# Cheng-Lin-Li/show-attend-and-tell

Measured on AMD Instinct MI355X. Metric: training images/sec, higher is better.
Workload: dtype bf16; 1 GPU; model=vgg16_frozen+attention_lstm512, global_batch=32, seq_len=20, vocab=5000, parallelism=dp1

## Files before the change

### sat_amd/models/encoders.py

```python

import torch
import torch.nn as tnn

from .nn import BatchNorm, Conv2d, MaxPool2d


class VGG16(tnn.Module):
    _PLAN = [
        ('conv1_1', 64), ('conv1_2', 64), 'pool',
        ('conv2_1', 128), ('conv2_2', 128), 'pool',
        ('conv3_1', 256), ('conv3_2', 256), ('conv3_3', 256), 'pool',
        ('conv4_1', 512), ('conv4_2', 512), ('conv4_3', 512), 'pool',
        ('conv5_1', 512), ('conv5_2', 512), ('conv5_3', 512),
    ]

    num_ctx = 196
    dim_ctx = 512

    def __init__(self, nn_policy):
        super().__init__()
        layers = []
        in_ch = 3
        for item in self._PLAN:
            if item == 'pool':
                layers.append(MaxPool2d(2, 2))
            else:
                name, out_ch = item
                conv = Conv2d(nn_policy, in_ch, out_ch, 3, 1, 'relu')
                self.add_module(name, conv)
                layers.append(conv)
                in_ch = out_ch
        self._layers = layers
        self.conv1_1._emit_padded = True
        self.conv1_2._accept_padded = True

    def forward(self, images):
        x = images
        for layer in self._layers:
            x = layer(x)
        return x.permute(0, 2, 3, 1).reshape(
            x.shape[0], -1, x.shape[1]).contiguous()


class _Bottleneck(tnn.Module):
    def __init__(self, nn_policy, in_ch, mid_ch, stride, project):
        super().__init__()
        out_ch = mid_ch * 4
        self.project = project
        if project:
            self.shortcut = Conv2d(nn_policy, in_ch, out_ch, 1, stride,
                                   None, use_bias=False)
            self.shortcut_bn = BatchNorm(nn_policy, out_ch)
        self.conv_a = Conv2d(nn_policy, in_ch, mid_ch, 1, stride, None,
                             use_bias=False)
        self.bn_a = BatchNorm(nn_policy, mid_ch)
        self.conv_b = Conv2d(nn_policy, mid_ch, mid_ch, 3, 1, None,
                             use_bias=False)
        self.bn_b = BatchNorm(nn_policy, mid_ch)
        self.conv_c = Conv2d(nn_policy, mid_ch, out_ch, 1, 1, None,
                             use_bias=False)
        self.bn_c = BatchNorm(nn_policy, out_ch)

    def forward(self, x):
        if self.project:
            sc = self.shortcut_bn(self.shortcut(x))
        else:
            sc = x
        y = self.bn_a(self.conv_a(x), relu=True)
        y = self.bn_b(self.conv_b(y), relu=True)
        y = self.bn_c(self.conv_c(y))
        return torch.relu(y + sc)


class ResNet50(tnn.Module):
    _STAGES = [(64, 3, 1), (128, 4, 2), (256, 6, 2), (512, 3, 2)]

    num_ctx = 49
    dim_ctx = 2048

    def __init__(self, nn_policy):
        super().__init__()
        self.conv1 = Conv2d(nn_policy, 3, 64, 7, 2, None, use_bias=False)
        self.bn1 = BatchNorm(nn_policy, 64)
        self.pool1 = MaxPool2d(3, 2)
        blocks = []
        in_ch = 64
        for s, (mid, n, stride) in enumerate(self._STAGES, start=2):
            for b in range(n):
                blk = _Bottleneck(nn_policy, in_ch, mid,
                                  stride if b == 0 else 1, b == 0)
                self.add_module('res%d%s' % (s, chr(ord('a') + b)), blk)
                blocks.append(blk)
                in_ch = mid * 4
        self._blocks = blocks

    def forward(self, images):
        x = self.bn1(self.conv1(images), relu=True)
        x = self.pool1(x)
        for blk in self._blocks:
            x = blk(x)
        return x.permute(0, 2, 3, 1).reshape(
            x.shape[0], -1, x.shape[1]).contiguous()


def build_encoder(name, nn_policy):
    if name == 'vgg16':
        return VGG16(nn_policy)
    if name == 'resnet50':
        return ResNet50(nn_policy)
    raise ValueError('unknown cnn %r' % (name,))
```

### sat_amd/models/nn.py

```python

import math

import torch
import torch.nn as tnn

from .. import ops


class NN(object):

    def __init__(self, config):
        self.config = config
        self.is_train = getattr(config, 'phase', 'train') == 'train'
        self.train_cnn = self.is_train and getattr(config, 'train_cnn', False)
        self.fc_scale = config.fc_kernel_initializer_scale
        self.fc_reg = config.fc_kernel_regularizer_scale \
            if self.is_train else 0.0
        self.conv_reg = config.conv_kernel_regularizer_scale \
            if self.train_cnn else 0.0
        self.fc_drop_rate = config.fc_drop_rate
        self.lstm_drop_rate = config.lstm_drop_rate
        self.fc_act_reg = getattr(
            config, 'fc_activity_regularizer_scale', 0.0) \
            if self.is_train else 0.0
        self.conv_act_reg = getattr(
            config, 'conv_activity_regularizer_scale', 0.0) \
            if self.train_cnn else 0.0
        self._regularized = []
        self._act_losses = []

    def init_fc_(self, t):
        tnn.init.uniform_(t, -self.fc_scale, self.fc_scale)

    def init_conv_(self, t):
        tnn.init.xavier_uniform_(t)

    def register_fc_kernel(self, p):
        if self.fc_reg > 0:
            self._regularized.append((p, self.fc_reg))

    def register_conv_kernel(self, p):
        if self.conv_reg > 0:
            self._regularized.append((p, self.conv_reg))

    def add_activity_loss(self, y, scale):
        if scale > 0 and torch.is_grad_enabled():
            self._act_losses.append(scale * y.float().abs().sum())

    def reg_loss(self):
        total = torch.zeros(())
        if self._regularized:
            if self._regularized[0][0].is_cuda:
                params = tuple(p for p, _ in self._regularized)
                scales = tuple(s for _, s in self._regularized)
                total = _RegL2.apply(scales, *params)
            else:
                total = sum(s * 0.5 * (p.float() ** 2).sum()
                            for p, s in self._regularized)
        if self._act_losses:
            act = sum(self._act_losses)
            self._act_losses = []
            total = total.to(act.device) + act
        return total

    def dropout(self, x):
        return ops.dropout(x, self.fc_drop_rate, self.is_train)


class _RegL2(torch.autograd.Function):

    _scale_cache = {}

    @staticmethod
    def forward(ctx, scales, *params):
        ctx.save_for_backward(*params)
        ctx.scales = scales
        norms = torch._foreach_norm(params, 2)
        sv = torch.stack([n.float() for n in norms])
        key = (scales, sv.device)
        sc = _RegL2._scale_cache.get(key)
        if sc is None:
            sc = torch.tensor(scales, dtype=torch.float32,
                              device=sv.device)
            _RegL2._scale_cache[key] = sc
        return (sv * sv * sc * 0.5).sum()

    @staticmethod
    def backward(ctx, d):
        params = ctx.saved_tensors
        gs = torch._foreach_mul(params, list(ctx.scales))
        gs = torch._foreach_mul(gs, d)
        return (None, *gs)


class Dense(tnn.Module):

    def __init__(self, nn_policy, in_dim, units, activation='tanh',
                 use_bias=True):
        super().__init__()
        self.activation = activation
        self._nn = nn_policy
        self.weight = tnn.Parameter(torch.empty(units, in_dim))
        nn_policy.init_fc_(self.weight)
        nn_policy.register_fc_kernel(self.weight)
        if use_bias:
            self.bias = tnn.Parameter(torch.zeros(units))
        else:
            self.register_parameter('bias', None)
        self._wc = None
        self._bc = None

    def precast(self, dtype):
        self._wc = self.weight.to(dtype)
        self._bc = self.bias.to(dtype) if self.bias is not None else None

    def clear_cast(self):
        self._wc = None
        self._bc = None

    def forward(self, x):
        if self._wc is not None and self._wc.dtype == x.dtype:
            y = ops.dense(x, self._wc, self._bc, self.activation)
        else:
            w = self.weight.to(x.dtype)
            b = self.bias.to(x.dtype) if self.bias is not None else None
            y = ops.dense(x, w, b, self.activation)
        if self.activation is not None and self._nn.fc_act_reg > 0:
            self._nn.add_activity_loss(y, self._nn.fc_act_reg)
        return y


class Conv2d(tnn.Module):

    def __init__(self, nn_policy, in_ch, out_ch, kernel_size=3, stride=1,
                 activation='relu', use_bias=True):
        super().__init__()
        self.stride = stride
        self.kernel_size = kernel_size
        self.activation = activation
        self._nn = nn_policy
        self._glds_conv = getattr(nn_policy.config, 'use_glds_conv',
                                  True)
        self.weight = tnn.Parameter(
            torch.empty(out_ch, in_ch, kernel_size, kernel_size))
        nn_policy.init_conv_(self.weight)
        nn_policy.register_conv_kernel(self.weight)
        if use_bias:
            self.bias = tnn.Parameter(torch.zeros(out_ch))
        else:
            self.register_parameter('bias', None)

    def forward(self, x):
        w = self.weight.to(x.dtype)
        b = self.bias.to(x.dtype) if self.bias is not None else None
        k, st = self.kernel_size, self.stride
        pad_hw = getattr(x, '_sat_pad', None)
        if pad_hw is not None and not (
                getattr(self, '_accept_padded', False)
                and k == 3 and st == 1
                and not torch.is_grad_enabled()):
            x = x[:, :, 1:-1, 1:-1] \
                .contiguous(memory_format=torch.channels_last)
            pad_hw = None
        if (torch.is_grad_enabled()
                and (x.requires_grad or w.requires_grad)
                and self._glds_conv and k == 3 and st == 1
                and self.activation in ('relu', None)):
            from ..ops.convgrad import Conv3x3Train, conv3x3_train_ok
            if conv3x3_train_ok(x, w):
                y = Conv3x3Train.apply(x, w, b,
                                       self.activation == 'relu')
                if self.activation is not None \
                        and self._nn.conv_act_reg > 0:
                    self._nn.add_activity_loss(y, self._nn.conv_act_reg)
                return y
        if (x.is_cuda and x.dtype == torch.bfloat16
                and not torch.is_grad_enabled()
                and k == 3 and st == 1 and w.shape[1] == 3
                and w.shape[0] % 8 == 0 and w.shape[0] <= 128
                and x.is_contiguous(memory_format=torch.channels_last)):
            from ..ops import hip
            if hip.available():
                from sat_amd import _C
                emit = bool(getattr(self, '_emit_padded', False)
                            and self._glds_conv)
                y = _C.conv3_fwd(
                    x, w.contiguous(),
                    b if b is not None
                    else torch.empty(0, dtype=x.dtype, device=x.device),
                    self.activation == 'relu', emit)
                if emit:
                    y._sat_pad = (x.shape[2], x.shape[3])
                return y
        if (x.is_cuda and x.dtype == torch.bfloat16
                and not torch.is_grad_enabled()
                and k == 3 and st == 1
                and w.shape[0] % 8 == 0 and w.shape[1] % 8 == 0
                and x.is_contiguous(memory_format=torch.channels_last)):
            from ..ops import hip
            if hip.available():
                from sat_amd import _C
                Cout, Cin = w.shape[0], w.shape[1]
                H = pad_hw[0] if pad_hw else x.shape[2]
                W = pad_hw[1] if pad_hw else x.shape[3]
                M = x.shape[0] * H * W
                relu = self.activation == 'relu'
                use_8p = (self._glds_conv and Cout % 256 == 0
                          and Cin % 64 == 0 and M >= 12544)
                use_glds = (self._glds_conv and not use_8p
                            and Cout >= 128 and Cout % 8 == 0
                            and Cin % 64 == 0 and Cin <= 128)
                use_g64 = (self._glds_conv and not use_8p
                           and not use_glds and Cout < 128
                           and Cin % 64 == 0)
                use_ig64 = (not use_8p and not use_glds and not use_g64
                            and Cin == 64 and pad_hw is None)
                if use_8p or use_glds or use_g64 or use_ig64:
                    if getattr(self, '_w_ohwi', None) is None or \
                            self._w_ohwi_ver != self.weight._version:
                        self._w_ohwi_ver = self.weight._version
                        self._w_ohwi = w.permute(0, 2, 3, 1).contiguous() \
                            .reshape(w.shape[0], -1)
                    eb = (b if b is not None else
                          torch.empty(0, dtype=x.dtype, device=x.device))
                    if use_ig64:
                        return _C.conv_igemm_fwd(x, self._w_ohwi, eb,
                                                 relu)
                    xp = x if pad_hw is not None else _C.pad1_nhwc(x)
                    if use_8p:
                        return _C.conv_igemm_8p_fwd(
                            xp, self._w_ohwi, eb, H, W, relu)
                    if use_glds:
                        return _C.conv_igemm_glds_fwd(
                            xp, self._w_ohwi, eb, H, W, relu)
                    return _C.conv_igemm_glds64_fwd(
                        xp, self._w_ohwi, eb, H, W, relu)
        if (x.is_cuda and x.dtype == torch.bfloat16
                and not torch.is_grad_enabled()
                and k == 1 and st == 1 and pad_hw is None
                and self._glds_conv
                and w.shape[0] % 8 == 0 and w.shape[1] % 8 == 0
                and x.is_contiguous(memory_format=torch.channels_last)):
            from ..ops import hip
            if hip.available():
                from sat_amd import _C
                B_, Cin, H, W = x.shape
                Cout = w.shape[0]
                rows = x.permute(0, 2, 3, 1).reshape(B_ * H * W, Cin)
                if getattr(self, '_w_1x1', None) is None or \
                        self._w_1x1_ver != self.weight._version:
                    self._w_1x1_ver = self.weight._version
                    self._w_1x1 = w.reshape(Cout, Cin).contiguous()
                eb = (b if b is not None else
                      torch.empty(0, dtype=x.dtype, device=x.device))
                act = 2 if self.activation == 'relu' else 0
                y = _C.dense_fwd(rows, self._w_1x1, eb, act)
                return y.reshape(B_, H, W, Cout).permute(0, 3, 1, 2)
        if pad_hw is not None:
            x = x[:, :, 1:-1, 1:-1] \
                .contiguous(memory_format=torch.channels_last)
        fuse_epi = (x.is_cuda and x.dtype == torch.bfloat16
                    and not torch.is_grad_enabled() and b is not None
                    and self.weight.shape[0] % 8 == 0)
        conv_bias = None if fuse_epi else b
        ph = _same_pad(x.shape[2], k, st)
        pw = _same_pad(x.shape[3], k, st)
        if ph % 2 == 0 and pw % 2 == 0:
            y = torch.nn.functional.conv2d(x, w, conv_bias, stride=st,
                                           padding=(ph // 2, pw // 2))
        else:
            x = torch.nn.functional.pad(
                x, (pw // 2, pw - pw // 2, ph // 2, ph - ph // 2))
            y = torch.nn.functional.conv2d(x, w, conv_bias, stride=st)
        if fuse_epi and y.is_contiguous(
                memory_format=torch.channels_last):
            from ..ops import hip
            if hip.available():
                from sat_amd import _C
                _C.bias_act_nhwc(y, b, self.activation == 'relu')
                return y
            y = y + b.reshape(1, -1, 1, 1)
        elif fuse_epi:
            y = y + b.reshape(1, -1, 1, 1)
        if self.activation == 'relu':
            y = torch.relu(y)
        if self.activation is not None and self._nn.conv_act_reg > 0:
            self._nn.add_activity_loss(y, self._nn.conv_act_reg)
        return y


def _same_pad(size, k, s):
    out = math.ceil(size / s)
    return max((out - 1) * s + k - size, 0)


def _pad_same(x, k, s):
    ph = _same_pad(x.shape[2], k, s)
    pw = _same_pad(x.shape[3], k, s)
    if ph == 0 and pw == 0:
        return x
    return torch.nn.functional.pad(
        x, (pw // 2, pw - pw // 2, ph // 2, ph - ph // 2))


class MaxPool2d(tnn.Module):

    def __init__(self, kernel_size=2, stride=2):
        super().__init__()
        self.kernel_size = kernel_size
        self.stride = stride

    def forward(self, x):
        if (x.is_cuda and x.dtype == torch.bfloat16
                and not torch.is_grad_enabled()
                and self.kernel_size == 2 and self.stride == 2
                and x.shape[1] % 8 == 0
                and x.is_contiguous(memory_format=torch.channels_last)):
            from ..ops import hip
            if hip.available():
                from sat_amd import _C
                return _C.maxpool2x2_nhwc(x)
        x = _pad_same(x, self.kernel_size, self.stride)
        return torch.nn.functional.max_pool2d(
            x, self.kernel_size, self.stride)


class BatchNorm(tnn.Module):

    def __init__(self, nn_policy, num_features):
        super().__init__()
        self.train_cnn = nn_policy.train_cnn
        self.bn = tnn.BatchNorm2d(num_features, eps=1e-3, momentum=0.01)
        self._ss = None

    def forward(self, x, relu=False):
        if self.train_cnn:
            y = self.bn(x.float()).to(x.dtype)
            return torch.relu(y) if relu else y
        if (x.is_cuda and x.dtype == torch.bfloat16
                and not torch.is_grad_enabled()
                and x.shape[1] % 8 == 0
                and x.is_contiguous(memory_format=torch.channels_last)):
            from ..ops import hip
            if hip.available():
                from sat_amd import _C
                ver = (self.bn.running_var._version,
                       self.bn.running_mean._version,
                       self.bn.weight._version,
                       self.bn.bias._version)
                if (self._ss is None or self._ss[0].device != x.device
                        or getattr(self, '_ss_ver', None) != ver):
                    self._ss_ver = ver
                    bn = self.bn
                    scale = (bn.weight /
                             torch.sqrt(bn.running_var + bn.eps))
                    shift = bn.bias - bn.running_mean * scale
                    self._ss = (scale.to(x.device, torch.bfloat16)
                                .contiguous(),
                                shift.to(x.device, torch.bfloat16)
                                .contiguous())
                _C.scale_bias_act_nhwc(x, self._ss[0], self._ss[1], relu)
                return x
        training = self.bn.training
        self.bn.eval()
        y = self.bn(x.float()).to(x.dtype)
        if training:
            self.bn.train()
        return torch.relu(y) if relu else y
```

### sat_amd/ops/csrc/bindings.cpp

```cpp
#include <torch/extension.h>
#include <vector>

at::Tensor dense_fwd(at::Tensor x, at::Tensor w, at::Tensor bias, int64_t act);
at::Tensor dense_fwd_drop(at::Tensor x, at::Tensor w, at::Tensor seed,
                          double p, int64_t salt);
std::vector<at::Tensor> dense_lstm_expand_fwd(
        at::Tensor xh, at::Tensor wl, at::Tensor bl, at::Tensor c_prev,
        at::Tensor pooled, at::Tensor table, at::Tensor ids,
        at::Tensor seed, at::Tensor expdrop, at::Tensor od_next,
        double fb, double p_lstm, double p_fc, int64_t s);
std::vector<at::Tensor> dexp_lstm_bwd(at::Tensor dexpd,
                                      at::Tensor d_out_carry,
                                      at::Tensor d_sth_carry,
                                      at::Tensor seed, at::Tensor gates,
                                      at::Tensor c_prev, at::Tensor dc,
                                      at::Tensor dgates_out,
                                      double p_fc, double p_lstm,
                                      int64_t s, int64_t D, int64_t E,
                                      double fb);
std::vector<at::Tensor> dense_dx_fuse(at::Tensor dgates, at::Tensor wl_t,
                                      at::Tensor dpool_dec,
                                      at::Tensor demb_dec,
                                      at::Tensor seed,
                                      at::Tensor demb_out,
                                      double p, int64_t salt,
                                      int64_t D, int64_t E, int64_t H);
at::Tensor conv3_fwd(at::Tensor input, at::Tensor weight, at::Tensor bias,
                     bool relu, bool emit_pad);
void bias_act_nhwc(at::Tensor y, at::Tensor bias, bool relu);
void scale_bias_act_nhwc(at::Tensor y, at::Tensor scale, at::Tensor shift,
                         bool relu);
at::Tensor maxpool2x2_nhwc(at::Tensor input);
at::Tensor conv_igemm_fwd(at::Tensor input, at::Tensor w_ohwi,
                          at::Tensor bias, bool relu);
at::Tensor pad1_nhwc(at::Tensor input);
at::Tensor conv_igemm_8p_fwd(at::Tensor padded, at::Tensor w_ohwi,
                             at::Tensor bias, int64_t Hh, int64_t Ww,
                             bool relu);
at::Tensor conv_igemm_glds64_fwd(at::Tensor padded, at::Tensor w_ohwi,
                                 at::Tensor bias, int64_t Hh, int64_t Ww,
                                 bool relu);
at::Tensor dense_8p_fwd(at::Tensor x, at::Tensor w, at::Tensor bias,
                        int64_t act);
at::Tensor conv3x3_wgrad(at::Tensor xpad, at::Tensor dy_rows,
                         int64_t Hh, int64_t Ww);
at::Tensor conv_igemm_glds_fwd(at::Tensor padded, at::Tensor w_ohwi,
                               at::Tensor bias, int64_t Hh, int64_t Ww,
                               bool relu);
std::vector<at::Tensor> dense_lstm_fwd(at::Tensor xh, at::Tensor wl,
                                       at::Tensor bl, at::Tensor c_prev,
                                       double fb);
std::vector<at::Tensor> lstm_pointwise_bwd_out(at::Tensor gates,
                                               at::Tensor c, at::Tensor dh,
                                               at::Tensor dc, double fb,
                                               at::Tensor dgates_out);
void lstm_in_fuse(at::Tensor pooled, at::Tensor table, at::Tensor ids,
                  at::Tensor sth, at::Tensor seed, double p, int64_t salt,
                  at::Tensor xh);
std::vector<at::Tensor> expand_fuse(at::Tensor h_raw, at::Tensor pooled,
                                    at::Tensor table, at::Tensor ids,
                                    at::Tensor seed,
                                    at::Tensor expdrop, at::Tensor od_next,
                                    double p_lstm, double p_fc, int64_t s);
std::vector<at::Tensor> dexp_fuse(at::Tensor dexpd, at::Tensor d_out_carry,
                                  at::Tensor d_sth_carry, at::Tensor seed,
                                  double p_fc, double p_lstm, int64_t s,
                                  int64_t D, int64_t E);
std::vector<at::Tensor> dx_fuse(at::Tensor dxh, at::Tensor dpool_dec,
                                at::Tensor demb_dec, at::Tensor seed,
                                at::Tensor demb_out, double p,
                                int64_t salt, int64_t H);
void hash_dropout_out(at::Tensor x, at::Tensor seed, double p,
                      int64_t salt, at::Tensor out);
at::Tensor hash_dropout_steps(at::Tensor x, at::Tensor seed, double p,
                              int64_t salt_base, int64_t salt_stride,
                              int64_t T);
void act_bwd_out(at::Tensor dy, at::Tensor y, int64_t act, at::Tensor out);
at::Tensor hash_dropout_slabs(at::Tensor x, at::Tensor seed, double p,
                              int64_t salt_base, int64_t salt_stride,
                              int64_t T);
std::vector<at::Tensor> lstm_pointwise_fwd(at::Tensor gates, at::Tensor c,
                                           double fb);
std::vector<at::Tensor> lstm_pointwise_bwd(at::Tensor gates, at::Tensor c,
                                           at::Tensor dh, at::Tensor dc,
                                           double fb);
at::Tensor act_bwd(at::Tensor dy, at::Tensor y, int64_t act);
void act_bwd_f32_out(at::Tensor dy, at::Tensor y, int64_t act,
                     at::Tensor out);
at::Tensor hash_dropout(at::Tensor x, at::Tensor seed, double p,
                        int64_t salt);
std::vector<at::Tensor> attn_pool_fwd(at::Tensor ctx, at::Tensor logits);
std::vector<at::Tensor> attn_scores_fused(at::Tensor t1, at::Tensor t2,
                                          at::Tensor v, at::Tensor seed,
                                          double p, int64_t salt, int64_t L);
std::vector<at::Tensor> attn_pool_bwd(at::Tensor ctx, at::Tensor alpha,
                                      at::Tensor dalpha, at::Tensor dpooled,
                                      bool need_dctx);
std::vector<at::Tensor> attn_scores_bwd(at::Tensor tdrop, at::Tensor v,
                                        at::Tensor dlogits, at::Tensor seed,
                                        double p, int64_t salt, int64_t L);
std::vector<at::Tensor> attn_scores_bwd_acc(at::Tensor tdrop, at::Tensor v,
                                            at::Tensor dlogits,
                                            at::Tensor seed, double p,
                                            int64_t salt, int64_t L,
                                            at::Tensor dv_acc);
std::vector<at::Tensor> attn_scores_bwd_tanh(
        at::Tensor tdrop, at::Tensor v, at::Tensor dlogits,
        at::Tensor seed, double p, int64_t salt, int64_t L,
        at::Tensor dv_acc, at::Tensor t1y, at::Tensor dt1_out);
at::Tensor embedding_fwd(at::Tensor ids, at::Tensor table);
at::Tensor embedding_bwd(at::Tensor ids, at::Tensor dy, int64_t rows);
std::vector<at::Tensor> ce_fwd(at::Tensor logits, at::Tensor labels,
                               at::Tensor mask);
at::Tensor ce_bwd(at::Tensor logits, at::Tensor labels, at::Tensor mask,
                  at::Tensor lse, at::Tensor dloss);
at::Tensor grad_sq_norm(std::vector<at::Tensor> grads);
at::Tensor sq_norm_mt(at::Tensor desc, at::Tensor cum, int64_t n_tensors,
                      int64_t total);
void adam_step_mt(at::Tensor desc, at::Tensor cum, int64_t n_tensors,
                  int64_t total, at::Tensor step_dev, double lr0,
                  double decay_factor, double steps_per_decay, double b1,
                  double b2, double eps, double clip, at::Tensor gsq,
                  bool zero_grads, bool vec4);
void adam_step(std::vector<at::Tensor> params, std::vector<at::Tensor> grads,
               std::vector<at::Tensor> ms, std::vector<at::Tensor> vs,
               at::Tensor step_dev, double lr0, double decay_factor,
               double steps_per_decay, double b1, double b2, double eps,
               double clip, at::Tensor gsq);

std::vector<at::Tensor> attn_scores_bwd_step(
    at::Tensor tdrop, at::Tensor v, at::Tensor dlogits, at::Tensor seed,
    double p, int64_t salt, int64_t L, at::Tensor dv_acc, at::Tensor t1y,
    at::Tensor dt1_out, at::Tensor dt2_out);
std::vector<at::Tensor> attn_pool_fwd_xh(at::Tensor ctx, at::Tensor logits,
                                         at::Tensor seed, double p,
                                         int64_t salt, at::Tensor xh,
                                         int64_t I);
void lstm_in_tail(at::Tensor table, at::Tensor ids, at::Tensor sth,
                  at::Tensor seed, double p, int64_t salt, at::Tensor xh,
                  int64_t D);
std::vector<at::Tensor> dense_lstm_expand_xh_fwd(
    at::Tensor xh, at::Tensor wl, at::Tensor bl, at::Tensor c_prev,
    at::Tensor pooled, at::Tensor table, at::Tensor ids, at::Tensor seed,
    at::Tensor expdrop, at::Tensor od_next, double fb, double p_lstm,
    double p_fc, int64_t s, at::Tensor next_ids, at::Tensor xh_next);
at::Tensor dense_tanhbwd_slabs(at::Tensor dy, at::Tensor y, at::Tensor w,
                               at::Tensor dpre_out);
at::Tensor slab_epilogue_drop(at::Tensor yf, at::Tensor seed, double p,
                              int64_t salt);
std::vector<at::Tensor> dexp_lstm_bwd_slabs(
    at::Tensor dexpd, at::Tensor carry_slabs, int64_t carry_salt,
    at::Tensor d_sth_carry, at::Tensor seed, at::Tensor gates,
    at::Tensor c_prev, at::Tensor dc, at::Tensor dgates_out, double p_fc,
    double p_lstm, int64_t s, int64_t D, int64_t E, double fb);

PYBIND11_MODULE(TORCH_EXTENSION_NAME, m) {
    m.def("dense_fwd", &dense_fwd, "MFMA GEMM + bias/act (bf16)");
    m.def("dense_fwd_drop", &dense_fwd_drop,
          "skinny GEMM with hash-dropout fused into the split-K epilogue");
    m.def("dense_lstm_expand_fwd", &dense_lstm_expand_fwd,
          "gates GEMM + LSTM gate math + expand scatter in 2 launches");
    m.def("dexp_lstm_bwd", &dexp_lstm_bwd,
          "dexp scatter + LSTM pointwise backward in one launch");
    m.def("dense_dx_fuse", &dense_dx_fuse,
          "dxh GEMM with the dx scatter fused into the epilogue");
    m.def("bias_act_nhwc", &bias_act_nhwc);
    m.def("scale_bias_act_nhwc", &scale_bias_act_nhwc);
    m.def("maxpool2x2_nhwc", &maxpool2x2_nhwc);
    m.def("conv_igemm_fwd", &conv_igemm_fwd);
    m.def("pad1_nhwc", &pad1_nhwc);
    m.def("conv_igemm_glds_fwd", &conv_igemm_glds_fwd);
    m.def("conv_igemm_8p_fwd", &conv_igemm_8p_fwd,
          "8-phase deep-pipelined implicit-GEMM conv (Cout%256==0)");
    m.def("conv_igemm_glds64_fwd", &conv_igemm_glds64_fwd);
    m.def("dense_8p_fwd", &dense_8p_fwd,
          "8-phase deep-pipelined dense GEMM (big-M shapes)");
    m.def("conv3x3_wgrad", &conv3x3_wgrad,
          "3x3 conv weight grad: transpose-staged MFMA split-K reduce");
    m.def("dense_lstm_fwd", &dense_lstm_fwd);
    m.def("conv3_fwd", &conv3_fwd,
          "direct NHWC conv for 3-channel 3x3/s1 (VGG conv1_1)");
    m.def("lstm_pointwise_bwd_out", &lstm_pointwise_bwd_out);
    m.def("lstm_in_fuse", &lstm_in_fuse);
    m.def("expand_fuse", &expand_fuse);
    m.def("dexp_fuse", &dexp_fuse);
    m.def("dx_fuse", &dx_fuse);
    m.def("hash_dropout_out", &hash_dropout_out);
    m.def("hash_dropout_steps", &hash_dropout_steps);
    m.def("act_bwd_out", &act_bwd_out);
    m.def("hash_dropout_slabs", &hash_dropout_slabs);
    m.def("lstm_pointwise_fwd", &lstm_pointwise_fwd);
    m.def("lstm_pointwise_bwd", &lstm_pointwise_bwd);
    m.def("act_bwd", &act_bwd);
    m.def("act_bwd_f32_out", &act_bwd_f32_out);
    m.def("hash_dropout", &hash_dropout);
    m.def("attn_pool_fwd", &attn_pool_fwd);
    m.def("attn_scores_fused", &attn_scores_fused);
    m.def("attn_pool_bwd", &attn_pool_bwd);
    m.def("attn_scores_bwd", &attn_scores_bwd);
    m.def("attn_scores_bwd_acc", &attn_scores_bwd_acc);
    m.def("attn_scores_bwd_tanh", &attn_scores_bwd_tanh,
          "scores backward with fused tanh-bwd dt1 into a given slab");
    m.def("embedding_fwd", &embedding_fwd);
    m.def("embedding_bwd", &embedding_bwd);
    m.def("ce_fwd", &ce_fwd);
    m.def("ce_bwd", &ce_bwd);
    m.def("grad_sq_norm", &grad_sq_norm);
    m.def("sq_norm_mt", &sq_norm_mt);
    m.def("adam_step_mt", &adam_step_mt);
    m.def("adam_step", &adam_step);
    m.def("attn_scores_bwd_step", &attn_scores_bwd_step,
          "attn_scores_bwd_tanh into a caller-zeroed dt2 slice");
    m.def("attn_pool_fwd_xh", &attn_pool_fwd_xh,
          "attention pool that also writes the dropped pooled columns "
          "of the LSTM input");
    m.def("lstm_in_tail", &lstm_in_tail,
          "embedding + state columns of the LSTM input (step 0)");
    m.def("dense_lstm_expand_xh_fwd", &dense_lstm_expand_xh_fwd,
          "dense_lstm_expand_fwd that also lays down the next step's "
          "embedding + state LSTM-input columns");
    m.def("dense_tanhbwd_slabs", &dense_tanhbwd_slabs,
          "split-K slabs of (dy * (1 - y^2)) @ w^T, tanh backward built "
          "in the A-operand load");
    m.def("slab_epilogue_drop", &slab_epilogue_drop,
          "bf16(sum of split-K slabs * dropout mask)");
    m.def("dexp_lstm_bwd_slabs", &dexp_lstm_bwd_slabs,
          "dexp_lstm_bwd taking d_out_carry as split-K slabs + salt");
}
```

### sat_amd/ops/csrc/common.h

```cpp
#pragma once

#include <hip/hip_runtime.h>
#include <hip/hip_bf16.h>
#include <torch/extension.h>
#include <ATen/cuda/CUDAContext.h>

#define CHECK_GPU(x) TORCH_CHECK((x).is_cuda(), #x " must be on GPU")
#define CHECK_CONTIG(x) TORCH_CHECK((x).is_contiguous(), #x " must be contiguous")
#define CHECK_BF16(x) TORCH_CHECK((x).scalar_type() == at::kBFloat16, #x " must be bf16")
#define CHECK_F32(x) TORCH_CHECK((x).scalar_type() == at::kFloat, #x " must be fp32")

#define HIP_OK(expr) do { hipError_t _e = (expr); \
    TORCH_CHECK(_e == hipSuccess, "HIP error: ", hipGetErrorString(_e)); } while (0)

using bf16 = __bf16;
typedef __attribute__((ext_vector_type(8))) __bf16 bf16x8;
typedef __attribute__((ext_vector_type(4))) float floatx4;

static inline int cdiv(int64_t a, int64_t b) { return (int)((a + b - 1) / b); }

__device__ __forceinline__ float bf2f(bf16 v) { return (float)v; }
__device__ __forceinline__ bf16 f2bf(float v) { return (bf16)v; }

__device__ __forceinline__ float wave_sum(float v) {
    for (int off = 32; off > 0; off >>= 1)
        v += __shfl_down(v, off, 64);
    return v;
}

__device__ __forceinline__ float wave_max(float v) {
    for (int off = 32; off > 0; off >>= 1)
        v = fmaxf(v, __shfl_down(v, off, 64));
    return v;
}

__device__ __forceinline__ float sigmoidf(float x) {
    return 1.0f / (1.0f + __expf(-x));
}

__device__ __forceinline__ uint32_t mix3(uint32_t a, uint32_t b, uint32_t c) {
    uint32_t h = a * 0x9E3779B1u ^ b * 0x85EBCA77u ^ c * 0xC2B2AE3Du;
    h ^= h >> 16; h *= 0x7FEB352Du;
    h ^= h >> 15; h *= 0x846CA68Bu;
    h ^= h >> 16;
    return h;
}

__device__ __forceinline__ float drop_scale(uint32_t seed, int salt,
                                            uint32_t idx, float p) {
    if (p <= 0.f) return 1.f;
    uint32_t h = mix3(seed, (uint32_t)salt, idx);
    float u = (h >> 8) * (1.0f / 16777216.0f);
    return u >= p ? 1.0f / (1.0f - p) : 0.0f;
}

__device__ __forceinline__ void drop_scale8(uint32_t seed, int salt,
                                            uint32_t idx8, float p,
                                            float* sc) {
    if (p <= 0.f) {
#pragma unroll
        for (int e = 0; e < 8; ++e) sc[e] = 1.f;
        return;
    }
    uint32_t pq = (uint32_t)(p * 256.0f);
    float inv = 1.0f / (1.0f - p);
    uint32_t h1 = mix3(seed, (uint32_t)salt, idx8);
    uint32_t h2 = mix3(h1, (uint32_t)salt ^ 0xA5A5A5A5u, idx8);
#pragma unroll
    for (int e = 0; e < 4; ++e) {
        sc[e] = ((h1 >> (e * 8)) & 0xFFu) >= pq ? inv : 0.f;
        sc[4 + e] = ((h2 >> (e * 8)) & 0xFFu) >= pq ? inv : 0.f;
    }
}

struct LstmAct { float gi, gj, gf, go, cn; };

__device__ __forceinline__ LstmAct lstm_act(const float g[4], float cp,
                                            float fb) {
#pragma clang fp contract(off)
    LstmAct a;
    a.gi = sigmoidf(g[0]);
    a.gj = tanhf(g[1]);
    a.gf = sigmoidf(g[2] + fb);
    a.go = sigmoidf(g[3]);
    a.cn = fmaf(a.gi, a.gj, cp * a.gf);
    return a;
}

__device__ __forceinline__ void lstm_cell_fwd(const float g[4], float cp,
                                              float fb, float& cn,
                                              float& h) {
    LstmAct a = lstm_act(g, cp, fb);
    cn = a.cn;
    h = tanhf(a.cn) * a.go;
}

__device__ __forceinline__ void lstm_cell_bwd(const float g[4], float cp,
                                              float dhv, float dcv,
                                              float fb, float dg[4],
                                              float& dcp) {
#pragma clang fp contract(off)
    LstmAct a = lstm_act(g, cp, fb);
    float tc = tanhf(a.cn);
    float dct = fmaf(dhv * a.go, 1.f - tc * tc, dcv);
    dg[0] = dct * a.gj * a.gi * (1.f - a.gi);
    dg[1] = dct * a.gi * fmaf(-a.gj, a.gj, 1.f);
    dg[2] = dct * cp * a.gf * (1.f - a.gf);
    dg[3] = dhv * tc * a.go * (1.f - a.go);
    dcp = dct * a.gf;
}

__device__ __forceinline__ float sum_slabs(const float* __restrict__ Yf,
                                           int64_t n, int64_t off,
                                           int splitk) {
    float v = 0.f;
    for (int k = 0; k < splitk; ++k) v += Yf[k * n + off];
    return v;
}
```

### sat_amd/ops/csrc/conv3.hip

```cpp

#include "common.h"

#define MAX_COUT 128
#ifndef LDS_STRIDE
#define LDS_STRIDE 72
#endif

__global__ __launch_bounds__(256)
void conv3_fwd_kernel(const bf16* __restrict__ in,
                      const bf16* __restrict__ w,
                      const bf16* __restrict__ bias,
                      bf16* __restrict__ out,
                      int BHW, int Hh, int Ww, int Cout, int relu,
                      int emit_pad) {
    __shared__ float ws[27 * MAX_COUT];
    __shared__ float bs[MAX_COUT];
    for (int i = threadIdx.x; i < 27 * Cout; i += blockDim.x) {
        int k = i / Cout, c = i % Cout;
        int ci = k / 9, ky = (k % 9) / 3, kx = k % 3;
        ws[i] = bf2f(w[((c * 3 + ci) * 3 + ky) * 3 + kx]);
    }
    for (int c = threadIdx.x; c < Cout; c += blockDim.x)
        bs[c] = (bias != nullptr) ? bf2f(bias[c]) : 0.f;
    __syncthreads();

    int pix = blockIdx.x * blockDim.x + threadIdx.x;
    if (pix >= BHW) return;
    int b = pix / (Hh * Ww);
    int yx = pix % (Hh * Ww);
    int y = yx / Ww, x = yx % Ww;

    float win[27];
#pragma unroll
    for (int ky = 0; ky < 3; ++ky) {
#pragma unroll
        for (int kx = 0; kx < 3; ++kx) {
            int yy = y + ky - 1, xx = x + kx - 1;
            bool ok = (yy >= 0 && yy < Hh && xx >= 0 && xx < Ww);
            const bf16* p = in + (((int64_t)b * Hh + yy) * Ww + xx) * 3;
#pragma unroll
            for (int ci = 0; ci < 3; ++ci)
                win[ci * 9 + ky * 3 + kx] = ok ? bf2f(p[ci]) : 0.f;
        }
    }

    bf16* op = emit_pad
        ? out + ((((int64_t)b * (Hh + 2) + y + 1) * (Ww + 2) + x + 1)
                 * Cout)
        : out + (int64_t)pix * Cout;
    for (int c0 = 0; c0 < Cout; c0 += 8) {
        bf16x8 o;
#pragma unroll
        for (int e = 0; e < 8; ++e) {
            int c = c0 + e;
            float acc = bs[c];
#pragma unroll
            for (int k = 0; k < 27; ++k)
                acc += win[k] * ws[k * Cout + c];
            if (relu) acc = fmaxf(acc, 0.f);
            o[e] = f2bf(acc);
        }
        *(bf16x8*)(op + c0) = o;
    }
}

__global__ void zero_border_kernel(bf16* __restrict__ out,
                                   int B, int Hp, int Wp, int C) {
    int64_t border = (int64_t)B * 2 * (Hp + Wp - 2);
    int64_t i = (int64_t)blockIdx.x * blockDim.x + threadIdx.x;
    int64_t n = border * (C / 8);
    if (i >= n) return;
    int c8 = (int)(i % (C / 8)) * 8;
    int64_t pb = i / (C / 8);
    int b = (int)(pb / (2 * (Hp + Wp - 2)));
    int q = (int)(pb % (2 * (Hp + Wp - 2)));
    int y, x;
    if (q < Wp) { y = 0; x = q; }
    else if (q < 2 * Wp) { y = Hp - 1; x = q - Wp; }
    else if (q < 2 * Wp + (Hp - 2)) { y = q - 2 * Wp + 1; x = 0; }
    else { y = q - 2 * Wp - (Hp - 2) + 1; x = Wp - 1; }
    bf16x8 z = {};
    *(bf16x8*)(out + (((int64_t)b * Hp + y) * Wp + x) * C + c8) = z;
}

at::Tensor conv3_fwd(at::Tensor input, at::Tensor weight, at::Tensor bias,
                     bool relu, bool emit_pad) {
    CHECK_GPU(input); CHECK_BF16(input);
    CHECK_GPU(weight); CHECK_BF16(weight);
    TORCH_CHECK(input.size(1) == 3 && weight.size(1) == 3
                && weight.size(2) == 3 && weight.size(3) == 3,
                "conv3_fwd: expects C_in=3, 3x3 kernel");
    TORCH_CHECK(input.is_contiguous(at::MemoryFormat::ChannelsLast),
                "conv3_fwd: input must be channels_last");
    int B = input.size(0), Hh = input.size(2), Ww = input.size(3);
    int Cout = weight.size(0);
    TORCH_CHECK(Cout % 8 == 0 && Cout <= MAX_COUT);
    auto wc = weight.contiguous();
    auto out = emit_pad
        ? at::empty({B, Cout, Hh + 2, Ww + 2},
                    input.options()
                        .memory_format(at::MemoryFormat::ChannelsLast))
        : at::empty({B, Cout, Hh, Ww},
                    input.options()
                        .memory_format(at::MemoryFormat::ChannelsLast));
    const bf16* bias_ptr = nullptr;
    if (bias.defined() && bias.numel() > 0)
        bias_ptr = (const bf16*)bias.contiguous().data_ptr();
    int BHW = B * Hh * Ww;
    hipStream_t s = at::cuda::getCurrentCUDAStream();
    if (emit_pad) {
        int64_t nb = (int64_t)B * 2 * (Hh + 2 + Ww + 2 - 2) * (Cout / 8);
        hipLaunchKernelGGL(zero_border_kernel, dim3(cdiv(nb, 256)),
                           dim3(256), 0, s,
                           (bf16*)out.data_ptr(), B, Hh + 2, Ww + 2,
                           Cout);
    }
    hipLaunchKernelGGL(conv3_fwd_kernel, dim3(cdiv(BHW, 256)), dim3(256),
                       0, s,
                       (const bf16*)input.data_ptr(),
                       (const bf16*)wc.data_ptr(), bias_ptr,
                       (bf16*)out.data_ptr(), BHW, Hh, Ww, Cout,
                       relu ? 1 : 0, emit_pad ? 1 : 0);
    HIP_OK(hipGetLastError());
    return out;
}


__global__ void bias_act_nhwc_kernel(bf16* __restrict__ y,
                                     const bf16* __restrict__ bias,
                                     int64_t n, int C, int relu) {
    int64_t i8 = ((int64_t)blockIdx.x * blockDim.x + threadIdx.x) * 8;
    if (i8 >= n) return;
    bf16x8 v = *(const bf16x8*)(y + i8);
    int c0 = (int)(i8 % C);
    const bf16x8 bv = *(const bf16x8*)(bias + c0);
#pragma unroll
    for (int e = 0; e < 8; ++e) {
        float t = bf2f(v[e]) + bf2f(bv[e]);
        if (relu) t = fmaxf(t, 0.f);
        v[e] = f2bf(t);
    }
    *(bf16x8*)(y + i8) = v;
}

void bias_act_nhwc(at::Tensor y, at::Tensor bias, bool relu) {
    CHECK_GPU(y); CHECK_BF16(y);
    int C = y.size(1);
    TORCH_CHECK(C % 8 == 0, "C must be a multiple of 8");
    TORCH_CHECK(y.is_contiguous(at::MemoryFormat::ChannelsLast));
    int64_t n = y.numel();
    hipStream_t s = at::cuda::getCurrentCUDAStream();
    hipLaunchKernelGGL(bias_act_nhwc_kernel, dim3(cdiv(n / 8, 256)),
                       dim3(256), 0, s,
                       (bf16*)y.data_ptr(),
                       (const bf16*)bias.contiguous().data_ptr(),
                       n, C, relu ? 1 : 0);
    HIP_OK(hipGetLastError());
}


__global__ void maxpool2x2_nhwc_kernel(const bf16* __restrict__ in,
                                       bf16* __restrict__ out,
                                       int B, int H, int W, int C,
                                       int Ho, int Wo) {
    int64_t i8 = ((int64_t)blockIdx.x * blockDim.x + threadIdx.x) * 8;
    int64_t n = (int64_t)B * Ho * Wo * C;
    if (i8 >= n) return;
    int c = (int)(i8 % C);
    int64_t pix = i8 / C;
    int xo = (int)(pix % Wo);
    int64_t t = pix / Wo;
    int yo = (int)(t % Ho);
    int b = (int)(t / Ho);
    int y0 = yo * 2, x0 = xo * 2;
    const bf16* base = in + (((int64_t)b * H + y0) * W + x0) * C + c;
    bf16x8 m = *(const bf16x8*)base;
    bf16x8 v;
    if (x0 + 1 < W) {
        v = *(const bf16x8*)(base + C);
#pragma unroll
        for (int e = 0; e < 8; ++e)
            if (bf2f(v[e]) > bf2f(m[e])) m[e] = v[e];
    }
    if (y0 + 1 < H) {
        v = *(const bf16x8*)(base + (int64_t)W * C);
#pragma unroll
        for (int e = 0; e < 8; ++e)
            if (bf2f(v[e]) > bf2f(m[e])) m[e] = v[e];
        if (x0 + 1 < W) {
            v = *(const bf16x8*)(base + (int64_t)W * C + C);
#pragma unroll
            for (int e = 0; e < 8; ++e)
                if (bf2f(v[e]) > bf2f(m[e])) m[e] = v[e];
        }
    }
    *(bf16x8*)(out + i8) = m;
}

at::Tensor maxpool2x2_nhwc(at::Tensor input) {
    CHECK_GPU(input); CHECK_BF16(input);
    TORCH_CHECK(input.is_contiguous(at::MemoryFormat::ChannelsLast));
    int B = input.size(0), C = input.size(1), H = input.size(2),
        W = input.size(3);
    TORCH_CHECK(C % 8 == 0);
    int Ho = (H + 1) / 2, Wo = (W + 1) / 2;
    auto out = at::empty({B, C, Ho, Wo},
                         input.options()
                             .memory_format(at::MemoryFormat::ChannelsLast));
    int64_t n = (int64_t)B * Ho * Wo * C;
    hipStream_t s = at::cuda::getCurrentCUDAStream();
    hipLaunchKernelGGL(maxpool2x2_nhwc_kernel, dim3(cdiv(n / 8, 256)),
                       dim3(256), 0, s,
                       (const bf16*)input.data_ptr(),
                       (bf16*)out.data_ptr(), B, H, W, C, Ho, Wo);
    HIP_OK(hipGetLastError());
    return out;
}


__global__ void scale_bias_act_nhwc_kernel(bf16* __restrict__ y,
                                           const bf16* __restrict__ scale,
                                           const bf16* __restrict__ shift,
                                           int64_t n, int C, int relu) {
    int64_t i8 = ((int64_t)blockIdx.x * blockDim.x + threadIdx.x) * 8;
    if (i8 >= n) return;
    bf16x8 v = *(const bf16x8*)(y + i8);
    int c0 = (int)(i8 % C);
    const bf16x8 sv = *(const bf16x8*)(scale + c0);
    const bf16x8 bv = *(const bf16x8*)(shift + c0);
#pragma unroll
    for (int e = 0; e < 8; ++e) {
        float t = bf2f(v[e]) * bf2f(sv[e]) + bf2f(bv[e]);
        if (relu) t = fmaxf(t, 0.f);
        v[e] = f2bf(t);
    }
    *(bf16x8*)(y + i8) = v;
}

void scale_bias_act_nhwc(at::Tensor y, at::Tensor scale, at::Tensor shift,
                         bool relu) {
    CHECK_GPU(y); CHECK_BF16(y);
    int C = y.size(1);
    TORCH_CHECK(C % 8 == 0, "C must be a multiple of 8");
    TORCH_CHECK(y.is_contiguous(at::MemoryFormat::ChannelsLast));
    int64_t n = y.numel();
    hipStream_t s = at::cuda::getCurrentCUDAStream();
    hipLaunchKernelGGL(scale_bias_act_nhwc_kernel, dim3(cdiv(n / 8, 256)),
                       dim3(256), 0, s,
                       (bf16*)y.data_ptr(),
                       (const bf16*)scale.data_ptr(),
                       (const bf16*)shift.data_ptr(),
                       n, C, relu ? 1 : 0);
    HIP_OK(hipGetLastError());
}


template <int WR, int WC, int FM, int FN>
__global__ __launch_bounds__(256)
void conv_igemm_kernel(const bf16* __restrict__ in,
                       const bf16* __restrict__ w,
                       const bf16* __restrict__ bias,
                       bf16* __restrict__ out,
                       int M, int Hh, int Ww, int Cin, int Cout,
                       int relu) {
    constexpr int BM = WR * FM * 16;
    constexpr int BN = WC * FN * 16;
    constexpr int BKc = 64;
    __shared__ bf16 As[BM * LDS_STRIDE];
    __shared__ bf16 Bs[BN * LDS_STRIDE];
    __shared__ int rbase[BM];
    __shared__ short rys[BM], rxs[BM];

    const int tid = threadIdx.x;
    const int lane = tid & 63;
    const int wave = tid >> 6;
    const int wr = wave / WC;
    const int wc = wave % WC;
    const int bm = blockIdx.y * BM;
    const int bn = blockIdx.x * BN;

    for (int r = tid; r < BM; r += blockDim.x) {
        int m = bm + r;
        if (m < M) {
            int b = m / (Hh * Ww);
            int yx = m % (Hh * Ww);
            int y = yx / Ww, x = yx % Ww;
            rbase[r] = ((b * Hh + y) * Ww + x) * Cin;
            rys[r] = (short)y;
            rxs[r] = (short)x;
        } else {
            rbase[r] = 0;
            rys[r] = -1;
            rxs[r] = -1;
        }
    }
    __syncthreads();

    floatx4 acc[FM][FN];
#pragma unroll
    for (int i = 0; i < FM; ++i)
#pragma unroll
        for (int j = 0; j < FN; ++j)
            acc[i][j] = floatx4{0.f, 0.f, 0.f, 0.f};

    const int lrow = lane & 15;
    const int kgrp = lane >> 4;
    const int KT = 9 * (Cin / BKc);
    constexpr int A_CHUNKS = BM * BKc / 8 / 256;
    constexpr int B_CHUNKS = BN * BKc / 8 / 256;

    for (int kt = 0; kt < KT; ++kt) {
        const int dxy = kt / (Cin / BKc);
        const int ci0 = (kt % (Cin / BKc)) * BKc;
        const int dy = dxy / 3 - 1, dx = dxy % 3 - 1;
        const int delta = (dy * Ww + dx) * Cin + ci0;

#pragma unroll
        for (int i = 0; i < A_CHUNKS; ++i) {
            int q = tid + 256 * i;
            int row = q >> 3;
            int c8 = (q & 7) * 8;
            int yy = rys[row] + dy, xx = rxs[row] + dx;
            bf16x8 v = {};
            if (yy >= 0 && yy < Hh && xx >= 0 && xx < Ww)
                v = *(const bf16x8*)(in + rbase[row] + delta + c8);
            *(bf16x8*)(As + row * LDS_STRIDE + c8) = v;
        }
#pragma unroll
        for (int i = 0; i < B_CHUNKS; ++i) {
            int q = tid + 256 * i;
            int row = q >> 3;
            int c8 = (q & 7) * 8;
            bf16x8 v = {};
            int gb = bn + row;
            if (gb < Cout)
                v = *(const bf16x8*)(
                    w + (int64_t)gb * 9 * Cin + dxy * Cin + ci0 + c8);
            *(bf16x8*)(Bs + row * LDS_STRIDE + c8) = v;
        }
        __syncthreads();

#pragma unroll
        for (int kk = 0; kk < 2; ++kk) {
            bf16x8 a_frag[FM], b_frag[FN];
            const int kof = kk * 32 + kgrp * 8;
#pragma unroll
            for (int mi = 0; mi < FM; ++mi)
                a_frag[mi] = *(const bf16x8*)(
                    As + (wr * FM * 16 + mi * 16 + lrow) * LDS_STRIDE
                    + kof);
#pragma unroll
            for (int ni = 0; ni < FN; ++ni)
                b_frag[ni] = *(const bf16x8*)(
                    Bs + (wc * FN * 16 + ni * 16 + lrow) * LDS_STRIDE
                    + kof);
#pragma unroll
            for (int mi = 0; mi < FM; ++mi)
#pragma unroll
                for (int ni = 0; ni < FN; ++ni)
                    acc[mi][ni] = __builtin_amdgcn_mfma_f32_16x16x32_bf16(
                        a_frag[mi], b_frag[ni], acc[mi][ni], 0, 0, 0);
        }
        __syncthreads();
    }

#pragma unroll
    for (int ni = 0; ni < FN; ++ni) {
        int col = bn + wc * FN * 16 + ni * 16 + (lane & 15);
        float bv = (bias != nullptr && col < Cout) ? bf2f(bias[col]) : 0.f;
#pragma unroll
        for (int mi = 0; mi < FM; ++mi) {
#pragma unroll
            for (int r = 0; r < 4; ++r) {
                int row = bm + wr * FM * 16 + mi * 16 + (lane >> 4) * 4
                    + r;
                if (row < M && col < Cout) {
                    float v = acc[mi][ni][r] + bv;
                    if (relu) v = fmaxf(v, 0.f);
                    out[(int64_t)row * Cout + col] = f2bf(v);
                }
            }
        }
    }
}

at::Tensor conv_igemm_fwd(at::Tensor input, at::Tensor w_ohwi,
                          at::Tensor bias, bool relu) {
    CHECK_GPU(input); CHECK_BF16(input);
    CHECK_GPU(w_ohwi); CHECK_CONTIG(w_ohwi); CHECK_BF16(w_ohwi);
    TORCH_CHECK(input.is_contiguous(at::MemoryFormat::ChannelsLast));
    int B = input.size(0), Cin = input.size(1), Hh = input.size(2),
        Ww = input.size(3);
    int Cout = w_ohwi.size(0);
    TORCH_CHECK(Cin % 64 == 0, "conv_igemm: Cin % 64 == 0");
    TORCH_CHECK(w_ohwi.numel() == (int64_t)Cout * 9 * Cin);
    auto out = at::empty({B, Cout, Hh, Ww},
                         input.options()
                             .memory_format(at::MemoryFormat::ChannelsLast));
    const bf16* bias_ptr = nullptr;
    if (bias.defined() && bias.numel() > 0)
        bias_ptr = (const bf16*)bias.contiguous().data_ptr();
    int M = B * Hh * Ww;
    hipStream_t s = at::cuda::getCurrentCUDAStream();
    if (Cout >= 128) {
        dim3 grid(cdiv(Cout, 128), cdiv(M, 128));
        hipLaunchKernelGGL((conv_igemm_kernel<2, 2, 4, 4>), grid,
                           dim3(256), 0, s,
                           (const bf16*)input.data_ptr(),
                           (const bf16*)w_ohwi.data_ptr(), bias_ptr,
                           (bf16*)out.data_ptr(), M, Hh, Ww, Cin, Cout,
                           relu ? 1 : 0);
    } else {
        dim3 grid(cdiv(Cout, 64), cdiv(M, 128));
        hipLaunchKernelGGL((conv_igemm_kernel<4, 1, 2, 4>), grid,
                           dim3(256), 0, s,
                           (const bf16*)input.data_ptr(),
                           (const bf16*)w_ohwi.data_ptr(), bias_ptr,
                           (bf16*)out.data_ptr(), M, Hh, Ww, Cin, Cout,
                           relu ? 1 : 0);
    }
    HIP_OK(hipGetLastError());
    return out;
}


__global__ void pad1_nhwc_kernel(const bf16* __restrict__ in,
                                 bf16* __restrict__ out,
                                 int B, int H, int W, int C) {
    int Hp = H + 2, Wp = W + 2;
    int64_t n = (int64_t)B * Hp * Wp * C;
    int64_t i8 = ((int64_t)blockIdx.x * blockDim.x + threadIdx.x) * 8;
    if (i8 >= n) return;
    int c = (int)(i8 % C);
    int64_t pix = i8 / C;
    int x = (int)(pix % Wp);
    int64_t t = pix / Wp;
    int y = (int)(t % Hp);
    int b = (int)(t / Hp);
    bf16x8 v = {};
    if (y >= 1 && y <= H && x >= 1 && x <= W)
        v = *(const bf16x8*)(in
                             + (((int64_t)b * H + y - 1) * W + x - 1) * C
                             + c);
    *(bf16x8*)(out + i8) = v;
}

at::Tensor pad1_nhwc(at::Tensor input) {
    CHECK_GPU(input); CHECK_BF16(input);
    TORCH_CHECK(input.is_contiguous(at::MemoryFormat::ChannelsLast));
    int B = input.size(0), C = input.size(1), H = input.size(2),
        W = input.size(3);
    TORCH_CHECK(C % 8 == 0);
    auto out = at::empty({B, C, H + 2, W + 2},
                         input.options()
                             .memory_format(at::MemoryFormat::ChannelsLast));
    int64_t n = (int64_t)B * (H + 2) * (W + 2) * C;
    hipStream_t s = at::cuda::getCurrentCUDAStream();
    hipLaunchKernelGGL(pad1_nhwc_kernel, dim3(cdiv(n / 8, 256)), dim3(256),
                       0, s,
                       (const bf16*)input.data_ptr(),
                       (bf16*)out.data_ptr(), B, H, W, C);
    HIP_OK(hipGetLastError());
    return out;
}

__global__ __launch_bounds__(256)
void conv_igemm_glds_kernel(const bf16* __restrict__ inp,
                            const bf16* __restrict__ w,
                            const bf16* __restrict__ bias,
                            bf16* __restrict__ out,
                            int M, int Hh, int Ww, int Cin, int Cout,
                            int relu) {
    constexpr int BM = 128, BN = 128, BKc = 64;
    __shared__ bf16 lds[2 * BM * BKc];
    bf16* As = lds;
    bf16* Bs = lds + BM * BKc;

    const int tid = threadIdx.x;
    const int lane = tid & 63;
    const int wave = tid >> 6;
    const int wr = wave >> 1, wc = wave & 1;
    const int bm = blockIdx.y * BM;
    const int bn = blockIdx.x * BN;
    const int Wp = Ww + 2;

    int aBase[4];
    int rowA[4];
#pragma unroll
    for (int i = 0; i < 4; ++i) {
        int r = wave * 32 + i * 8 + (lane >> 3);
        rowA[i] = r;
        int m = bm + r;
        if (m >= M) m = M - 1;
        int b = m / (Hh * Ww);
        int yx = m % (Hh * Ww);
        int y = yx / Ww, x = yx % Ww;
        aBase[i] = ((b * (Hh + 2) + y + 1) * Wp + x + 1) * Cin;
    }
    const bf16* wBase[4];
#pragma unroll
    for (int i = 0; i < 4; ++i) {
        int cout = bn + wave * 32 + i * 8 + (lane >> 3);
        if (cout >= Cout) cout = Cout - 1;
        wBase[i] = w + (int64_t)cout * 9 * Cin;
    }
    const int ci8 = (lane & 7) * 8;

    floatx4 acc[4][4];
#pragma unroll
    for (int i = 0; i < 4; ++i)
#pragma unroll
        for (int j = 0; j < 4; ++j)
            acc[i][j] = floatx4{0.f, 0.f, 0.f, 0.f};

    const int lrow = lane & 15;
    const int kgrp = lane >> 4;
    const int KT = 9 * (Cin / BKc);

    for (int kt = 0; kt < KT; ++kt) {
        const int dxy = kt / (Cin / BKc);
        const int ci0 = (kt % (Cin / BKc)) * BKc;
        const int dy = dxy / 3 - 1, dx = dxy % 3 - 1;
        const int delta = (dy * Wp + dx) * Cin + ci0 + ci8;

#pragma unroll
        for (int i = 0; i < 4; ++i) {
            int swz = (rowA[i] & 4) ? 16 : 0;
            __builtin_amdgcn_global_load_lds(
                (const __attribute__((address_space(1))) uint32_t*)
                    (inp + aBase[i] + delta + (ci8 ^ swz) - ci8),
                (__attribute__((address_space(3))) uint32_t*)
                    (As + (wave * 32 + i * 8) * BKc),
                16, 0, 0);
            __builtin_amdgcn_global_load_lds(
                (const __attribute__((address_space(1))) uint32_t*)
                    (wBase[i] + dxy * Cin + ci0 + (ci8 ^ swz)),
                (__attribute__((address_space(3))) uint32_t*)
                    (Bs + (wave * 32 + i * 8) * BKc),
                16, 0, 0);
        }
        __syncthreads();

#pragma unroll
        for (int kk = 0; kk < 2; ++kk) {
            bf16x8 a_frag[4], b_frag[4];
            const int kof = kk * 32 + kgrp * 8;
#pragma unroll
            for (int mi = 0; mi < 4; ++mi) {
                int r = wr * 64 + mi * 16 + lrow;
                a_frag[mi] = *(const bf16x8*)(
                    As + r * BKc + (kof ^ ((r & 4) ? 16 : 0)));
            }
#pragma unroll
            for (int ni = 0; ni < 4; ++ni) {
                int r = wc * 64 + ni * 16 + lrow;
                b_frag[ni] = *(const bf16x8*)(
                    Bs + r * BKc + (kof ^ ((r & 4) ? 16 : 0)));
            }
#pragma unroll
            for (int mi = 0; mi < 4; ++mi)
#pragma unroll
                for (int ni = 0; ni < 4; ++ni)
                    acc[mi][ni] = __builtin_amdgcn_mfma_f32_16x16x32_bf16(
                        a_frag[mi], b_frag[ni], acc[mi][ni], 0, 0, 0);
        }
        __syncthreads();
    }

#pragma unroll
    for (int ni = 0; ni < 4; ++ni) {
        int col = bn + wc * 64 + ni * 16 + (lane & 15);
        float bv = (bias != nullptr && col < Cout) ? bf2f(bias[col]) : 0.f;
#pragma unroll
        for (int mi = 0; mi < 4; ++mi) {
#pragma unroll
            for (int r = 0; r < 4; ++r) {
                int row = bm + wr * 64 + mi * 16 + (lane >> 4) * 4 + r;
                if (row < M && col < Cout) {
                    float vv = acc[mi][ni][r] + bv;
                    if (relu) vv = fmaxf(vv, 0.f);
                    out[(int64_t)row * Cout + col] = f2bf(vv);
                }
            }
        }
    }
}

at::Tensor conv_igemm_glds_fwd(at::Tensor padded, at::Tensor w_ohwi,
                               at::Tensor bias, int64_t Hh, int64_t Ww,
                               bool relu) {
    CHECK_GPU(padded); CHECK_BF16(padded);
    CHECK_GPU(w_ohwi); CHECK_CONTIG(w_ohwi); CHECK_BF16(w_ohwi);
    TORCH_CHECK(padded.is_contiguous(at::MemoryFormat::ChannelsLast));
    int B = padded.size(0), Cin = padded.size(1);
    TORCH_CHECK(padded.size(2) == Hh + 2 && padded.size(3) == Ww + 2);
    int Cout = w_ohwi.size(0);
    TORCH_CHECK(Cin % 64 == 0 && Cout % 8 == 0);
    auto out = at::empty({B, Cout, Hh, Ww},
                         padded.options()
                             .memory_format(at::MemoryFormat::ChannelsLast));
    const bf16* bias_ptr = nullptr;
    if (bias.defined() && bias.numel() > 0)
        bias_ptr = (const bf16*)bias.contiguous().data_ptr();
    int M = B * Hh * Ww;
    dim3 grid(cdiv(Cout, 128), cdiv(M, 128));
    hipStream_t s = at::cuda::getCurrentCUDAStream();
    hipLaunchKernelGGL(conv_igemm_glds_kernel, grid, dim3(256), 0, s,
                       (const bf16*)padded.data_ptr(),
                       (const bf16*)w_ohwi.data_ptr(), bias_ptr,
                       (bf16*)out.data_ptr(), (int)M, (int)Hh, (int)Ww,
                       (int)Cin, (int)Cout, relu ? 1 : 0);
    HIP_OK(hipGetLastError());
    return out;
}


__global__ __launch_bounds__(256)
void conv_igemm_glds64_kernel(const bf16* __restrict__ inp,
                              const bf16* __restrict__ w,
                              const bf16* __restrict__ bias,
                              bf16* __restrict__ out,
                              int M, int Hh, int Ww, int Cin, int Cout,
                              int relu) {
    constexpr int BM = 128, BKc = 64;
    __shared__ bf16 lds[(BM + 64) * BKc];
    bf16* As = lds;
    bf16* Bs = lds + BM * BKc;

    const int tid = threadIdx.x;
    const int lane = tid & 63;
    const int wave = tid >> 6;
    const int bm = blockIdx.y * BM;
    const int bn = blockIdx.x * 64;
    const int Wp = Ww + 2;

    int aBase[4];
    int rowA[4];
#pragma unroll
    for (int i = 0; i < 4; ++i) {
        int r = wave * 32 + i * 8 + (lane >> 3);
        rowA[i] = r;
        int m = bm + r;
        if (m >= M) m = M - 1;
        int b = m / (Hh * Ww);
        int yx = m % (Hh * Ww);
        int y = yx / Ww, x = yx % Ww;
        aBase[i] = ((b * (Hh + 2) + y + 1) * Wp + x + 1) * Cin;
    }
    const bf16* wBase[2];
    int rowB[2];
#pragma unroll
    for (int j = 0; j < 2; ++j) {
        int r = wave * 16 + j * 8 + (lane >> 3);
        rowB[j] = r;
        int cout = bn + r;
        if (cout >= Cout) cout = Cout - 1;
        wBase[j] = w + (int64_t)cout * 9 * Cin;
    }
    const int ci8 = (lane & 7) * 8;

    floatx4 acc[2][4];
#pragma unroll
    for (int i = 0; i < 2; ++i)
#pragma unroll
        for (int j = 0; j < 4; ++j)
            acc[i][j] = floatx4{0.f, 0.f, 0.f, 0.f};

    const int lrow = lane & 15;
    const int kgrp = lane >> 4;
    const int KT = 9 * (Cin / BKc);

    for (int kt = 0; kt < KT; ++kt) {
        const int dxy = kt / (Cin / BKc);
        const int ci0 = (kt % (Cin / BKc)) * BKc;
        const int dy = dxy / 3 - 1, dx = dxy % 3 - 1;
        const int delta = (dy * Wp + dx) * Cin + ci0 + ci8;

#pragma unroll
        for (int i = 0; i < 4; ++i) {
            int swz = (rowA[i] & 4) ? 16 : 0;
            __builtin_amdgcn_global_load_lds(
                (const __attribute__((address_space(1))) uint32_t*)
                    (inp + aBase[i] + delta + (ci8 ^ swz) - ci8),
                (__attribute__((address_space(3))) uint32_t*)
                    (As + (wave * 32 + i * 8) * BKc),
                16, 0, 0);
        }
#pragma unroll
        for (int j = 0; j < 2; ++j) {
            int swz = (rowB[j] & 4) ? 16 : 0;
            __builtin_amdgcn_global_load_lds(
                (const __attribute__((address_space(1))) uint32_t*)
                    (wBase[j] + dxy * Cin + ci0 + (ci8 ^ swz)),
                (__attribute__((address_space(3))) uint32_t*)
                    (Bs + (wave * 16 + j * 8) * BKc),
                16, 0, 0);
        }
        __syncthreads();

#pragma unroll
        for (int kk = 0; kk < 2; ++kk) {
            bf16x8 a_frag[2], b_frag[4];
            const int kof = kk * 32 + kgrp * 8;
#pragma unroll
            for (int mi = 0; mi < 2; ++mi) {
                int r = wave * 32 + mi * 16 + lrow;
                a_frag[mi] = *(const bf16x8*)(
                    As + r * BKc + (kof ^ ((r & 4) ? 16 : 0)));
            }
#pragma unroll
            for (int ni = 0; ni < 4; ++ni) {
                int r = ni * 16 + lrow;
                b_frag[ni] = *(const bf16x8*)(
                    Bs + r * BKc + (kof ^ ((r & 4) ? 16 : 0)));
            }
#pragma unroll
            for (int mi = 0; mi < 2; ++mi)
#pragma unroll
                for (int ni = 0; ni < 4; ++ni)
                    acc[mi][ni] = __builtin_amdgcn_mfma_f32_16x16x32_bf16(
                        a_frag[mi], b_frag[ni], acc[mi][ni], 0, 0, 0);
        }
        __syncthreads();
    }

#pragma unroll
    for (int ni = 0; ni < 4; ++ni) {
        int col = bn + ni * 16 + (lane & 15);
        float bv = (bias != nullptr && col < Cout) ? bf2f(bias[col]) : 0.f;
#pragma unroll
        for (int mi = 0; mi < 2; ++mi) {
#pragma unroll
            for (int r = 0; r < 4; ++r) {
                int row = bm + wave * 32 + mi * 16 + (lane >> 4) * 4 + r;
                if (row < M && col < Cout) {
                    float vv = acc[mi][ni][r] + bv;
                    if (relu) vv = fmaxf(vv, 0.f);
                    out[(int64_t)row * Cout + col] = f2bf(vv);
                }
            }
        }
    }
}

at::Tensor conv_igemm_glds64_fwd(at::Tensor padded, at::Tensor w_ohwi,
                                 at::Tensor bias, int64_t Hh, int64_t Ww,
                                 bool relu) {
    CHECK_GPU(padded); CHECK_BF16(padded);
    CHECK_GPU(w_ohwi); CHECK_CONTIG(w_ohwi); CHECK_BF16(w_ohwi);
    TORCH_CHECK(padded.is_contiguous(at::MemoryFormat::ChannelsLast));
    int B = padded.size(0), Cin = padded.size(1);
    TORCH_CHECK(padded.size(2) == Hh + 2 && padded.size(3) == Ww + 2);
    int Cout = w_ohwi.size(0);
    TORCH_CHECK(Cin % 64 == 0 && Cout % 8 == 0);
    auto out = at::empty({B, Cout, Hh, Ww},
                         padded.options()
                             .memory_format(at::MemoryFormat::ChannelsLast));
    const bf16* bias_ptr = nullptr;
    if (bias.defined() && bias.numel() > 0)
        bias_ptr = (const bf16*)bias.contiguous().data_ptr();
    int M = B * Hh * Ww;
    dim3 grid(cdiv(Cout, 64), cdiv(M, 128));
    hipStream_t s = at::cuda::getCurrentCUDAStream();
    hipLaunchKernelGGL(conv_igemm_glds64_kernel, grid, dim3(256), 0, s,
                       (const bf16*)padded.data_ptr(),
                       (const bf16*)w_ohwi.data_ptr(), bias_ptr,
                       (bf16*)out.data_ptr(), (int)M, (int)Hh, (int)Ww,
                       (int)Cin, (int)Cout, relu ? 1 : 0);
    HIP_OK(hipGetLastError());
    return out;
}
```

### sat_amd/ops/csrc/conv8p.hip

```cpp

#include "common.h"

namespace {

constexpr int SLOT = 8192;

__device__ __forceinline__ void glds16(const bf16* src, bf16* dst) {
    __builtin_amdgcn_global_load_lds(
        (const __attribute__((address_space(1))) uint32_t*)src,
        (__attribute__((address_space(3))) uint32_t*)dst, 16, 0, 0);
}

__device__ __forceinline__ int swz16(int row) {
    return (row & 4) ? 16 : 0;
}

}

template <int SPLIT>
__global__ __launch_bounds__(512)
void conv_igemm_8p_kernel(const bf16* __restrict__ inp,
                          const bf16* __restrict__ w,
                          const bf16* __restrict__ bias,
                          bf16* __restrict__ out,
                          float* __restrict__ outf,
                          int M, int Hh, int Ww, int Cin, int Cout,
                          int relu, int kt_per) {
    __shared__ bf16 lds[8 * SLOT];

    const int tid = threadIdx.x;
    const int lane = tid & 63;
    const int wave = tid >> 6;
    const int wr = wave >> 2;
    const int wc = wave & 3;
    const int bm = blockIdx.y * 256;
    const int bn = blockIdx.x * 256;
    const int Wp = Ww + 2;

    const int srow = wave * 8 + (lane >> 3);
    const int selem = (lane & 7) * 8;
    const bf16* aSrc[2][2];
    const bf16* bSrc[2][2];
#pragma unroll
    for (int h = 0; h < 2; ++h) {
#pragma unroll
        for (int j = 0; j < 2; ++j) {
            int r = j * 64 + srow;
            int m = bm + h * 128 + r;
            if (m >= M) m = M - 1;
            int b = m / (Hh * Ww);
            int yx = m % (Hh * Ww);
            int y = yx / Ww, x = yx % Ww;
            aSrc[h][j] = inp
                + (((int64_t)b * (Hh + 2) + y + 1) * Wp + x + 1) * Cin
                + (selem ^ swz16(r));
            int cb = bn + h * 128 + r;
            if (cb >= Cout) cb = Cout - 1;
            bSrc[h][j] = w + (int64_t)cb * 9 * Cin + (selem ^ swz16(r));
        }
    }
    bf16* dstJ0 = lds + (wave * 8) * 64;
    bf16* dstJ1 = lds + (64 + wave * 8) * 64;

    const int KT = 9 * (Cin / 64);
    const int kt0 = SPLIT ? blockIdx.z * kt_per : 0;
    const int kt1 = SPLIT ? min(kt0 + kt_per, KT) : KT;

    const int CT = Cin / 64;

#define A_DELTA(kt) ((((kt) / CT) / 3 - 1) * Wp + ((kt) / CT) % 3 - 1) \
        * Cin + ((kt) % CT) * 64
#define B_DELTA(kt) ((kt) / CT) * Cin + ((kt) % CT) * 64

#define STAGE(kt, h) do {                                               \
        int _slot = (((kt) & 1) * 4 + (h));                             \
        bf16* _d0 = dstJ0 + _slot * SLOT;                               \
        bf16* _d1 = dstJ1 + _slot * SLOT;                               \
        if ((h) == 0)      { glds16(aSrc[0][0] + A_DELTA(kt), _d0);     \
                             glds16(aSrc[0][1] + A_DELTA(kt), _d1); }   \
        else if ((h) == 1) { glds16(bSrc[0][0] + B_DELTA(kt), _d0);     \
                             glds16(bSrc[0][1] + B_DELTA(kt), _d1); }   \
        else if ((h) == 2) { glds16(aSrc[1][0] + A_DELTA(kt), _d0);     \
                             glds16(aSrc[1][1] + A_DELTA(kt), _d1); }   \
        else               { glds16(bSrc[1][0] + B_DELTA(kt), _d0);     \
                             glds16(bSrc[1][1] + B_DELTA(kt), _d1); }   \
    } while (0)

    floatx4 acc[8][4];
#pragma unroll
    for (int i = 0; i < 8; ++i)
#pragma unroll
        for (int j = 0; j < 4; ++j)
            acc[i][j] = floatx4{0.f, 0.f, 0.f, 0.f};

    const int lrow = lane & 15;
    const int kgrp = lane >> 4;

#define READ_A(dst, kt, aH) do {                                        \
        const bf16* _s = lds + ((((kt) & 1) * 4 + ((aH) ? 2 : 0)))      \
            * SLOT;                                                     \
        _Pragma("unroll")                                               \
        for (int mi = 0; mi < 4; ++mi) {                                \
            int _r = wr * 64 + mi * 16 + lrow;                          \
            _Pragma("unroll")                                           \
            for (int kk = 0; kk < 2; ++kk)                              \
                dst[mi][kk] = *(const bf16x8*)(                         \
                    _s + _r * 64 + ((kk * 32 + kgrp * 8)                \
                                    ^ swz16(_r)));                      \
        }                                                               \
    } while (0)
#define READ_B(dst, kt, bH) do {                                        \
        const bf16* _s = lds + ((((kt) & 1) * 4 + ((bH) ? 3 : 1)))      \
            * SLOT;                                                     \
        _Pragma("unroll")                                               \
        for (int ni = 0; ni < 2; ++ni) {                                \
            int _r = wc * 32 + ni * 16 + lrow;                          \
            _Pragma("unroll")                                           \
            for (int kk = 0; kk < 2; ++kk)                              \
                dst[ni][kk] = *(const bf16x8*)(                         \
                    _s + _r * 64 + ((kk * 32 + kgrp * 8)                \
                                    ^ swz16(_r)));                      \
        }                                                               \
    } while (0)

#define MFMA16(aH, bH) do {                                             \
        __builtin_amdgcn_s_setprio(1);                                  \
        _Pragma("unroll")                                               \
        for (int mi = 0; mi < 4; ++mi)                                  \
            _Pragma("unroll")                                           \
            for (int ni = 0; ni < 2; ++ni)                              \
                _Pragma("unroll")                                       \
                for (int kk = 0; kk < 2; ++kk)                          \
                    acc[(aH) * 4 + mi][(bH) * 2 + ni] =                 \
                        __builtin_amdgcn_mfma_f32_16x16x32_bf16(        \
                            afr[mi][kk], bfr[ni][kk],                   \
                            acc[(aH) * 4 + mi][(bH) * 2 + ni], 0, 0, 0);\
        __builtin_amdgcn_s_setprio(0);                                  \
    } while (0)

#define VMW(n) asm volatile("s_waitcnt vmcnt(" #n ")" ::: "memory")
#define BAR() __builtin_amdgcn_s_barrier()
#define LGKM0() asm volatile("s_waitcnt lgkmcnt(0)" ::: "memory")

    bf16x8 afr[4][2], bfr[2][2];

    STAGE(kt0, 0); STAGE(kt0, 1); STAGE(kt0, 2); STAGE(kt0, 3);
    VMW(4); BAR();

    for (int t = kt0; t + 1 < kt1; ++t) {
        READ_A(afr, t, 0); READ_B(bfr, t, 0);
        STAGE(t + 1, 0);
        VMW(4); BAR(); LGKM0();
        MFMA16(0, 0);
        BAR();
        READ_A(afr, t, 1);
        STAGE(t + 1, 1);
        VMW(4); BAR(); LGKM0();
        MFMA16(1, 0);
        BAR();
        READ_B(bfr, t, 1);
        STAGE(t + 1, 2);
        VMW(4); BAR(); LGKM0();
        MFMA16(1, 1);
        BAR();
        READ_A(afr, t, 0);
        STAGE(t + 1, 3);
        VMW(4); BAR(); LGKM0();
        MFMA16(0, 1);
        BAR();
    }

    VMW(0); BAR();
    {
        const int t = kt1 - 1;
        READ_A(afr, t, 0); READ_B(bfr, t, 0); LGKM0();
        MFMA16(0, 0);
        READ_A(afr, t, 1); LGKM0();
        MFMA16(1, 0);
        READ_B(bfr, t, 1); LGKM0();
        MFMA16(1, 1);
        READ_A(afr, t, 0); LGKM0();
        MFMA16(0, 1);
    }

#undef STAGE
#undef READ_A
#undef READ_B
#undef MFMA16
#undef VMW
#undef BAR
#undef LGKM0
#undef A_DELTA
#undef B_DELTA

#pragma unroll
    for (int bH = 0; bH < 2; ++bH) {
#pragma unroll
        for (int ni = 0; ni < 2; ++ni) {
            int col = bn + bH * 128 + wc * 32 + ni * 16 + (lane & 15);
            float bv = (!SPLIT && bias != nullptr && col < Cout)
                ? bf2f(bias[col]) : 0.f;
#pragma unroll
            for (int aH = 0; aH < 2; ++aH) {
#pragma unroll
                for (int mi = 0; mi < 4; ++mi) {
#pragma unroll
                    for (int r = 0; r < 4; ++r) {
                        int row = bm + aH * 128 + wr * 64 + mi * 16
                            + (lane >> 4) * 4 + r;
                        if (row < M && col < Cout) {
                            if (SPLIT) {
                                atomicAdd(
                                    outf + (int64_t)row * Cout + col,
                                    acc[aH * 4 + mi][bH * 2 + ni][r]);
                            } else {
                                float v = acc[aH * 4 + mi]
                                    [bH * 2 + ni][r] + bv;
                                if (relu) v = fmaxf(v, 0.f);
                                out[(int64_t)row * Cout + col]
                                    = f2bf(v);
                            }
                        }
                    }
                }
            }
        }
    }
}

__global__ void f32_bias_act_nhwc_kernel(const float* __restrict__ yf,
                                         const bf16* __restrict__ bias,
                                         bf16* __restrict__ out,
                                         int64_t n, int C, int relu) {
    int64_t i8 = ((int64_t)blockIdx.x * blockDim.x + threadIdx.x) * 8;
    if (i8 >= n) return;
    int c0 = (int)(i8 % C);
#pragma unroll
    for (int e = 0; e < 8; ++e) {
        float t = yf[i8 + e];
        if (bias != nullptr) t += bf2f(bias[c0 + e]);
        if (relu) t = fmaxf(t, 0.f);
        out[i8 + e] = f2bf(t);
    }
}

at::Tensor conv_igemm_8p_fwd(at::Tensor padded, at::Tensor w_ohwi,
                             at::Tensor bias, int64_t Hh, int64_t Ww,
                             bool relu) {
    CHECK_GPU(padded); CHECK_BF16(padded);
    CHECK_GPU(w_ohwi); CHECK_CONTIG(w_ohwi); CHECK_BF16(w_ohwi);
    TORCH_CHECK(padded.is_contiguous(at::MemoryFormat::ChannelsLast));
    int B = padded.size(0), Cin = padded.size(1);
    TORCH_CHECK(padded.size(2) == Hh + 2 && padded.size(3) == Ww + 2);
    int Cout = w_ohwi.size(0);
    TORCH_CHECK(Cin % 64 == 0 && Cin >= 64, "conv_igemm_8p: Cin % 64");
    TORCH_CHECK(Cout % 256 == 0, "conv_igemm_8p: Cout % 256");
    TORCH_CHECK(w_ohwi.numel() == (int64_t)Cout * 9 * Cin);
    auto out = at::empty({B, Cout, Hh, Ww},
                         padded.options()
                             .memory_format(at::MemoryFormat::ChannelsLast));
    const bf16* bias_ptr = nullptr;
    if (bias.defined() && bias.numel() > 0)
        bias_ptr = (const bf16*)bias.contiguous().data_ptr();
    int64_t M64 = (int64_t)B * Hh * Ww;
    TORCH_CHECK(M64 < (1LL << 31), "conv_igemm_8p: M too large");
    int M = (int)M64;
    int blocks = cdiv(Cout, 256) * cdiv(M, 256);
    int KT = 9 * (Cin / 64);
    int splitz = std::max(1, std::min({8, 224 / blocks, KT / 2}));
    hipStream_t s = at::cuda::getCurrentCUDAStream();
    if (splitz > 1) {
        auto scratch = at::zeros({M, Cout},
                                 padded.options().dtype(at::kFloat));
        int kt_per = cdiv(KT, splitz);
        splitz = cdiv(KT, kt_per);
        dim3 grid(cdiv(Cout, 256), cdiv(M, 256), splitz);
        hipLaunchKernelGGL((conv_igemm_8p_kernel<1>), grid, dim3(512),
                           0, s,
                           (const bf16*)padded.data_ptr(),
                           (const bf16*)w_ohwi.data_ptr(), bias_ptr,
                           nullptr, (float*)scratch.data_ptr(),
                           M, (int)Hh, (int)Ww,
                           (int)Cin, (int)Cout, relu ? 1 : 0, kt_per);
        int64_t n = (int64_t)M * Cout;
        hipLaunchKernelGGL(f32_bias_act_nhwc_kernel,
                           dim3(cdiv(n / 8, 256)), dim3(256), 0, s,
                           (const float*)scratch.data_ptr(), bias_ptr,
                           (bf16*)out.data_ptr(), n, (int)Cout,
                           relu ? 1 : 0);
    } else {
        dim3 grid(cdiv(Cout, 256), cdiv(M, 256));
        hipLaunchKernelGGL((conv_igemm_8p_kernel<0>), grid, dim3(512),
                           0, s,
                           (const bf16*)padded.data_ptr(),
                           (const bf16*)w_ohwi.data_ptr(), bias_ptr,
                           (bf16*)out.data_ptr(), nullptr,
                           M, (int)Hh, (int)Ww,
                           (int)Cin, (int)Cout, relu ? 1 : 0, KT);
    }
    HIP_OK(hipGetLastError());
    return out;
}
```

Baseline: 5880 images/sec.

## Chain padded NHWC outputs through VGG conv and pool layers

Extends the padded-output path from conv1_1 to every VGG conv/maxpool producer whose consumer is an implicit-GEMM 3x3 conv. Each producer writes directly into a halo-padded buffer and zeroes the border in its epilogue, so the separate pad1_nhwc copy and the zero-border kernel go away. The 8p split-K path also routes its bias/act epilogue through the padded layout, and the threshold for the 8p route is lowered under the default setting so more layers use it. The cost is extra epilogue address arithmetic and border writes, plus more complex routing logic.

```diff
diff --git a/sat_amd/models/encoders.py b/sat_amd/models/encoders.py
--- a/sat_amd/models/encoders.py
+++ b/sat_amd/models/encoders.py
@@ -31,8 +31,11 @@
                 layers.append(conv)
                 in_ch = out_ch
         self._layers = layers
-        self.conv1_1._emit_padded = True
-        self.conv1_2._accept_padded = True
+        for prod, cons in zip(layers[:-1], layers[1:]):
+            if isinstance(cons, Conv2d) and cons.weight.shape[1] % 64 == 0:
+                prod._emit_padded = True
+                prod._pad_consumer_ok = cons._accepts_padded
+                cons._accept_padded = True
 
     def forward(self, images):
         x = images
diff --git a/sat_amd/models/nn.py b/sat_amd/models/nn.py
--- a/sat_amd/models/nn.py
+++ b/sat_amd/models/nn.py
@@ -5,6 +5,23 @@
 import torch.nn as tnn
 
 from .. import ops
+
+PAD_CHAIN = True
+
+PAD_CHAIN_8P = False
+
+CONV5_ROUTE = 'intree'
+_8P_FULL_M = 12544
+_8P_SPLIT_M = 6272
+
+
+def _8p_single_pass(Cout, Cin, M):
+    blocks = -(-Cout // 256) * -(-M // 256)
+    return min(8, 224 // blocks, 9 * (Cin // 64) // 2) <= 1
+
+
+def _unpad(x):
+    return x[:, :, 1:-1, 1:-1].contiguous(memory_format=torch.channels_last)
 
 
 class NN(object):
@@ -150,6 +167,35 @@
         else:
             self.register_parameter('bias', None)
 
+    def _igemm_route(self, M, padded_in=False):
+        Cout, Cin = self.weight.shape[0], self.weight.shape[1]
+        if (self.kernel_size != 3 or self.stride != 1
+                or Cout % 8 != 0 or Cin % 8 != 0):
+            return None
+        if self._glds_conv and Cin % 64 == 0:
+            min_m = _8P_SPLIT_M if CONV5_ROUTE == 'intree' else _8P_FULL_M
+            if Cout % 256 == 0 and M >= min_m:
+                return '8p'
+            if Cout >= 128 and Cin <= 128:
+                return 'glds'
+            if Cout < 128:
+                return 'g64'
+        if Cin == 64 and not padded_in:
+            return 'ig64'
+        return None
+
+    def _accepts_padded(self, M):
+        return (getattr(self, '_accept_padded', False)
+                and self._igemm_route(M, True) in ('8p', 'glds', 'g64'))
+
+    def _emits_padded(self, M):
+        if not (getattr(self, '_emit_padded', False) and self._glds_conv):
+            return False
+        if not (PAD_CHAIN or self.weight.shape[1] == 3):
+            return False
+        ok = getattr(self, '_pad_consumer_ok', None)
+        return ok is None or ok(M)
+
     def forward(self, x):
         w = self.weight.to(x.dtype)
         b = self.bias.to(x.dtype) if self.bias is not None else None
@@ -159,8 +205,7 @@
                 getattr(self, '_accept_padded', False)
                 and k == 3 and st == 1
                 and not torch.is_grad_enabled()):
-            x = x[:, :, 1:-1, 1:-1] \
-                .contiguous(memory_format=torch.channels_last)
+            x = _unpad(x)
             pad_hw = None
         if (torch.is_grad_enabled()
                 and (x.requires_grad or w.requires_grad)
@@ -182,8 +227,8 @@
             from ..ops import hip
             if hip.available():
                 from sat_amd import _C
-                emit = bool(getattr(self, '_emit_padded', False)
-                            and self._glds_conv)
+                emit = self._emits_padded(
+                    x.shape[0] * x.shape[2] * x.shape[3])
                 y = _C.conv3_fwd(
                     x, w.contiguous(),
                     b if b is not None
@@ -200,22 +245,12 @@
             from ..ops import hip
             if hip.available():
                 from sat_amd import _C
-                Cout, Cin = w.shape[0], w.shape[1]
                 H = pad_hw[0] if pad_hw else x.shape[2]
                 W = pad_hw[1] if pad_hw else x.shape[3]
                 M = x.shape[0] * H * W
                 relu = self.activation == 'relu'
-                use_8p = (self._glds_conv and Cout % 256 == 0
-                          and Cin % 64 == 0 and M >= 12544)
-                use_glds = (self._glds_conv and not use_8p
-                            and Cout >= 128 and Cout % 8 == 0
-                            and Cin % 64 == 0 and Cin <= 128)
-                use_g64 = (self._glds_conv and not use_8p
-                           and not use_glds and Cout < 128
-                           and Cin % 64 == 0)
-                use_ig64 = (not use_8p and not use_glds and not use_g64
-                            and Cin == 64 and pad_hw is None)
-                if use_8p or use_glds or use_g64 or use_ig64:
+                route = self._igemm_route(M, pad_hw is not None)
+                if route is not None:
                     if getattr(self, '_w_ohwi', None) is None or \
                             self._w_ohwi_ver != self.weight._version:
                         self._w_ohwi_ver = self.weight._version
@@ -223,18 +258,20 @@
                             .reshape(w.shape[0], -1)
                     eb = (b if b is not None else
                           torch.empty(0, dtype=x.dtype, device=x.device))
-                    if use_ig64:
+                    if route == 'ig64':
                         return _C.conv_igemm_fwd(x, self._w_ohwi, eb,
                                                  relu)
                     xp = x if pad_hw is not None else _C.pad1_nhwc(x)
-                    if use_8p:
-                        return _C.conv_igemm_8p_fwd(
-                            xp, self._w_ohwi, eb, H, W, relu)
-                    if use_glds:
-                        return _C.conv_igemm_glds_fwd(
-                            xp, self._w_ohwi, eb, H, W, relu)
-                    return _C.conv_igemm_glds64_fwd(
-                        xp, self._w_ohwi, eb, H, W, relu)
+                    emit = self._emits_padded(M) and (
+                        route != '8p' or PAD_CHAIN_8P
+                        or not _8p_single_pass(w.shape[0], w.shape[1], M))
+                    fwd = {'8p': _C.conv_igemm_8p_fwd,
+                           'glds': _C.conv_igemm_glds_fwd,
+                           'g64': _C.conv_igemm_glds64_fwd}[route]
+                    y = fwd(xp, self._w_ohwi, eb, H, W, relu, emit)
+                    if emit:
+                        y._sat_pad = (H, W)
+                    return y
         if (x.is_cuda and x.dtype == torch.bfloat16
                 and not torch.is_grad_enabled()
                 and k == 1 and st == 1 and pad_hw is None
@@ -311,6 +348,8 @@
         self.stride = stride
 
     def forward(self, x):
+        if getattr(x, '_sat_pad', None) is not None:
+            x = _unpad(x)
         if (x.is_cuda and x.dtype == torch.bfloat16
                 and not torch.is_grad_enabled()
                 and self.kernel_size == 2 and self.stride == 2
@@ -319,7 +358,16 @@
             from ..ops import hip
             if hip.available():
                 from sat_amd import _C
-                return _C.maxpool2x2_nhwc(x)
+                Ho, Wo = (x.shape[2] + 1) // 2, (x.shape[3] + 1) // 2
+                ok = getattr(self, '_pad_consumer_ok', None)
+                emit = bool(PAD_CHAIN
+                            and getattr(self, '_emit_padded', False)
+                            and ok is not None
+                            and ok(x.shape[0] * Ho * Wo))
+                y = _C.maxpool2x2_nhwc(x, emit)
+                if emit:
+                    y._sat_pad = (Ho, Wo)
+                return y
         x = _pad_same(x, self.kernel_size, self.stride)
         return torch.nn.functional.max_pool2d(
             x, self.kernel_size, self.stride)
diff --git a/sat_amd/ops/csrc/bindings.cpp b/sat_amd/ops/csrc/bindings.cpp
--- a/sat_amd/ops/csrc/bindings.cpp
+++ b/sat_amd/ops/csrc/bindings.cpp
@@ -26,27 +26,32 @@
                                       double p, int64_t salt,
                                       int64_t D, int64_t E, int64_t H);
 at::Tensor conv3_fwd(at::Tensor input, at::Tensor weight, at::Tensor bias,
-                     bool relu, bool emit_pad);
+                     bool relu, bool emit_pad,
+                     c10::optional<at::Tensor> out);
 void bias_act_nhwc(at::Tensor y, at::Tensor bias, bool relu);
 void scale_bias_act_nhwc(at::Tensor y, at::Tensor scale, at::Tensor shift,
                          bool relu);
-at::Tensor maxpool2x2_nhwc(at::Tensor input);
+at::Tensor maxpool2x2_nhwc(at::Tensor input, bool emit_pad,
+                           c10::optional<at::Tensor> out);
 at::Tensor conv_igemm_fwd(at::Tensor input, at::Tensor w_ohwi,
                           at::Tensor bias, bool relu);
 at::Tensor pad1_nhwc(at::Tensor input);
 at::Tensor conv_igemm_8p_fwd(at::Tensor padded, at::Tensor w_ohwi,
                              at::Tensor bias, int64_t Hh, int64_t Ww,
-                             bool relu);
+                             bool relu, bool emit_pad,
+                             c10::optional<at::Tensor> out, int64_t split);
 at::Tensor conv_igemm_glds64_fwd(at::Tensor padded, at::Tensor w_ohwi,
                                  at::Tensor bias, int64_t Hh, int64_t Ww,
-                                 bool relu);
+                                 bool relu, bool emit_pad,
+                                 c10::optional<at::Tensor> out);
 at::Tensor dense_8p_fwd(at::Tensor x, at::Tensor w, at::Tensor bias,
                         int64_t act);
 at::Tensor conv3x3_wgrad(at::Tensor xpad, at::Tensor dy_rows,
                          int64_t Hh, int64_t Ww);
 at::Tensor conv_igemm_glds_fwd(at::Tensor padded, at::Tensor w_ohwi,
                                at::Tensor bias, int64_t Hh, int64_t Ww,
-                               bool relu);
+                               bool relu, bool emit_pad,
+                               c10::optional<at::Tensor> out);
 std::vector<at::Tensor> dense_lstm_fwd(at::Tensor xh, at::Tensor wl,
                                        at::Tensor bl, at::Tensor c_prev,
                                        double fb);
@@ -154,6 +159,10 @@
     at::Tensor c_prev, at::Tensor dc, at::Tensor dgates_out, double p_fc,
     double p_lstm, int64_t s, int64_t D, int64_t E, double fb);
 
+#define CONV_ARGS py::arg("padded"), py::arg("w_ohwi"), py::arg("bias"), \
+    py::arg("H"), py::arg("W"), py::arg("relu"),                         \
+    py::arg("emit_pad") = false, py::arg("out") = py::none()
+
 PYBIND11_MODULE(TORCH_EXTENSION_NAME, m) {
     m.def("dense_fwd", &dense_fwd, "MFMA GEMM + bias/act (bf16)");
     m.def("dense_fwd_drop", &dense_fwd_drop,
@@ -166,20 +175,26 @@
           "dxh GEMM with the dx scatter fused into the epilogue");
     m.def("bias_act_nhwc", &bias_act_nhwc);
     m.def("scale_bias_act_nhwc", &scale_bias_act_nhwc);
-    m.def("maxpool2x2_nhwc", &maxpool2x2_nhwc);
+    m.def("maxpool2x2_nhwc", &maxpool2x2_nhwc, py::arg("input"),
+          py::arg("emit_pad") = false, py::arg("out") = py::none());
     m.def("conv_igemm_fwd", &conv_igemm_fwd);
     m.def("pad1_nhwc", &pad1_nhwc);
-    m.def("conv_igemm_glds_fwd", &conv_igemm_glds_fwd);
+    m.def("conv_igemm_glds_fwd", &conv_igemm_glds_fwd, CONV_ARGS);
     m.def("conv_igemm_8p_fwd", &conv_igemm_8p_fwd,
-          "8-phase deep-pipelined implicit-GEMM conv (Cout%256==0)");
-    m.def("conv_igemm_glds64_fwd", &conv_igemm_glds64_fwd);
+          "8-phase deep-pipelined implicit-GEMM conv (Cout%256==0); "
+          "split: -1 auto, 0 single pass, >= 2 that many K slices",
+          CONV_ARGS, py::arg("split") = -1);
+    m.def("conv_igemm_glds64_fwd", &conv_igemm_glds64_fwd, CONV_ARGS);
     m.def("dense_8p_fwd", &dense_8p_fwd,
           "8-phase deep-pipelined dense GEMM (big-M shapes)");
     m.def("conv3x3_wgrad", &conv3x3_wgrad,
           "3x3 conv weight grad: transpose-staged MFMA split-K reduce");
     m.def("dense_lstm_fwd", &dense_lstm_fwd);
     m.def("conv3_fwd", &conv3_fwd,
-          "direct NHWC conv for 3-channel 3x3/s1 (VGG conv1_1)");
+          "direct NHWC conv for 3-channel 3x3/s1 (VGG conv1_1)",
+          py::arg("input"), py::arg("weight"), py::arg("bias"),
+          py::arg("relu"), py::arg("emit_pad"),
+          py::arg("out") = py::none());
     m.def("lstm_pointwise_bwd_out", &lstm_pointwise_bwd_out);
     m.def("lstm_in_fuse", &lstm_in_fuse);
     m.def("expand_fuse", &expand_fuse);
diff --git a/sat_amd/ops/csrc/common.h b/sat_amd/ops/csrc/common.h
--- a/sat_amd/ops/csrc/common.h
+++ b/sat_amd/ops/csrc/common.h
@@ -110,6 +110,89 @@
     dcp = dct * a.gf;
 }
 
+
+struct PadPix { int pix, y, x; };
+
+__device__ __forceinline__ PadPix pad_pix(int m, int H, int W) {
+    int b = m / (H * W);
+    int yx = m - b * (H * W);
+    PadPix p;
+    p.y = yx / W;
+    p.x = yx - p.y * W;
+    p.pix = (b * (H + 2) + p.y + 1) * (W + 2) + p.x + 1;
+    return p;
+}
+
+__device__ __forceinline__ void pad_pix_next(PadPix& p, int H, int W) {
+    const bool wx = (p.x + 1 == W);
+    const bool wy = wx && (p.y + 1 == H);
+    p.pix += 1 + (wx ? 2 : 0) + (wy ? 2 * (W + 2) : 0);
+    p.y = wy ? 0 : (wx ? p.y + 1 : p.y);
+    p.x = wx ? 0 : p.x + 1;
+}
+
+template <typename T>
+__device__ __forceinline__ void pad_border_zero(bf16* p, int y, int x,
+                                                int H, int W, int C) {
+    const bool l = (x == 0), r = (x == W - 1);
+    if (!(l || r || y == 0 || y == H - 1)) return;
+    const int64_t rs = (int64_t)(W + 2) * C;
+    const T z = {};
+    if (l) *(T*)(p - C) = z;
+    if (r) *(T*)(p + C) = z;
+    if (y == 0) {
+        *(T*)(p - rs) = z;
+        if (l) *(T*)(p - rs - C) = z;
+        if (r) *(T*)(p - rs + C) = z;
+    }
+    if (y == H - 1) {
+        *(T*)(p + rs) = z;
+        if (l) *(T*)(p + rs - C) = z;
+        if (r) *(T*)(p + rs + C) = z;
+    }
+}
+
+__device__ __forceinline__ void pad_border_run(bf16* out, int row0, int M,
+                                               int H, int W, int C,
+                                               const int (&cols)[4]) {
+    if (row0 >= M) return;
+    PadPix p = pad_pix(row0, H, W);
+#pragma unroll 1
+    for (int r = 0; r < 4 && row0 + r < M; ++r) {
+        if (r) pad_pix_next(p, H, W);
+        if (p.x == 0 || p.x == W - 1 || p.y == 0 || p.y == H - 1) {
+            bf16* q = out + (int64_t)p.pix * C;
+#pragma unroll 1
+            for (int j = 0; j < 4; ++j)
+                if (cols[j] < C)
+                    pad_border_zero<bf16>(q + cols[j], p.y, p.x, H, W, C);
+        }
+    }
+}
+
+static inline at::Tensor nhwc_out(const at::Tensor& like, int64_t B,
+                                  int64_t C, int64_t H, int64_t W,
+                                  bool emit_pad,
+                                  const c10::optional<at::Tensor>& out) {
+    const int64_t Ho = emit_pad ? H + 2 : H, Wo = emit_pad ? W + 2 : W;
+    TORCH_CHECK(B * Ho * Wo < (1LL << 31), "output has >= 2^31 pixels");
+    if (out.has_value() && out->defined()) {
+        CHECK_GPU(*out); CHECK_BF16(*out);
+        TORCH_CHECK(out->dim() == 4 && out->size(0) == B
+                    && out->size(1) == C && out->size(2) == Ho
+                    && out->size(3) == Wo,
+                    "out: expected [", B, ",", C, ",", Ho, ",", Wo, "]");
+        TORCH_CHECK(out->is_contiguous(at::MemoryFormat::ChannelsLast),
+                    "out must be channels_last");
+        TORCH_CHECK(out->device() == like.device(),
+                    "out must be on the input's device");
+        return *out;
+    }
+    return at::empty({B, C, Ho, Wo},
+                     like.options()
+                         .memory_format(at::MemoryFormat::ChannelsLast));
+}
+
 __device__ __forceinline__ float sum_slabs(const float* __restrict__ Yf,
                                            int64_t n, int64_t off,
                                            int splitk) {
diff --git a/sat_amd/ops/csrc/conv3.hip b/sat_amd/ops/csrc/conv3.hip
--- a/sat_amd/ops/csrc/conv3.hip
+++ b/sat_amd/ops/csrc/conv3.hip
@@ -48,6 +48,9 @@
         ? out + ((((int64_t)b * (Hh + 2) + y + 1) * (Ww + 2) + x + 1)
                  * Cout)
         : out + (int64_t)pix * Cout;
+    if (emit_pad)
+        for (int c0 = 0; c0 < Cout; c0 += 8)
+            pad_border_zero<bf16x8>(op + c0, y, x, Hh, Ww, Cout);
     for (int c0 = 0; c0 < Cout; c0 += 8) {
         bf16x8 o;
 #pragma unroll
@@ -64,27 +67,9 @@
     }
 }
 
-__global__ void zero_border_kernel(bf16* __restrict__ out,
-                                   int B, int Hp, int Wp, int C) {
-    int64_t border = (int64_t)B * 2 * (Hp + Wp - 2);
-    int64_t i = (int64_t)blockIdx.x * blockDim.x + threadIdx.x;
-    int64_t n = border * (C / 8);
-    if (i >= n) return;
-    int c8 = (int)(i % (C / 8)) * 8;
-    int64_t pb = i / (C / 8);
-    int b = (int)(pb / (2 * (Hp + Wp - 2)));
-    int q = (int)(pb % (2 * (Hp + Wp - 2)));
-    int y, x;
-    if (q < Wp) { y = 0; x = q; }
-    else if (q < 2 * Wp) { y = Hp - 1; x = q - Wp; }
-    else if (q < 2 * Wp + (Hp - 2)) { y = q - 2 * Wp + 1; x = 0; }
-    else { y = q - 2 * Wp - (Hp - 2) + 1; x = Wp - 1; }
-    bf16x8 z = {};
-    *(bf16x8*)(out + (((int64_t)b * Hp + y) * Wp + x) * C + c8) = z;
-}
-
 at::Tensor conv3_fwd(at::Tensor input, at::Tensor weight, at::Tensor bias,
-                     bool relu, bool emit_pad) {
+                     bool relu, bool emit_pad,
+                     c10::optional<at::Tensor> out_opt) {
     CHECK_GPU(input); CHECK_BF16(input);
     CHECK_GPU(weight); CHECK_BF16(weight);
     TORCH_CHECK(input.size(1) == 3 && weight.size(1) == 3
@@ -96,25 +81,12 @@
     int Cout = weight.size(0);
     TORCH_CHECK(Cout % 8 == 0 && Cout <= MAX_COUT);
     auto wc = weight.contiguous();
-    auto out = emit_pad
-        ? at::empty({B, Cout, Hh + 2, Ww + 2},
-                    input.options()
-                        .memory_format(at::MemoryFormat::ChannelsLast))
-        : at::empty({B, Cout, Hh, Ww},
-                    input.options()
-                        .memory_format(at::MemoryFormat::ChannelsLast));
+    auto out = nhwc_out(input, B, Cout, Hh, Ww, emit_pad, out_opt);
     const bf16* bias_ptr = nullptr;
     if (bias.defined() && bias.numel() > 0)
         bias_ptr = (const bf16*)bias.contiguous().data_ptr();
     int BHW = B * Hh * Ww;
     hipStream_t s = at::cuda::getCurrentCUDAStream();
-    if (emit_pad) {
-        int64_t nb = (int64_t)B * 2 * (Hh + 2 + Ww + 2 - 2) * (Cout / 8);
-        hipLaunchKernelGGL(zero_border_kernel, dim3(cdiv(nb, 256)),
-                           dim3(256), 0, s,
-                           (bf16*)out.data_ptr(), B, Hh + 2, Ww + 2,
-                           Cout);
-    }
     hipLaunchKernelGGL(conv3_fwd_kernel, dim3(cdiv(BHW, 256)), dim3(256),
                        0, s,
                        (const bf16*)input.data_ptr(),
@@ -162,7 +134,7 @@
 __global__ void maxpool2x2_nhwc_kernel(const bf16* __restrict__ in,
                                        bf16* __restrict__ out,
                                        int B, int H, int W, int C,
-                                       int Ho, int Wo) {
+                                       int Ho, int Wo, int emit_pad) {
     int64_t i8 = ((int64_t)blockIdx.x * blockDim.x + threadIdx.x) * 8;
     int64_t n = (int64_t)B * Ho * Wo * C;
     if (i8 >= n) return;
@@ -194,25 +166,33 @@
                 if (bf2f(v[e]) > bf2f(m[e])) m[e] = v[e];
         }
     }
-    *(bf16x8*)(out + i8) = m;
-}
-
-at::Tensor maxpool2x2_nhwc(at::Tensor input) {
+    if (emit_pad) {
+        bf16* op = out
+            + (((int64_t)b * (Ho + 2) + yo + 1) * (Wo + 2) + xo + 1) * C
+            + c;
+        *(bf16x8*)op = m;
+        pad_border_zero<bf16x8>(op, yo, xo, Ho, Wo, C);
+    } else {
+        *(bf16x8*)(out + i8) = m;
+    }
+}
+
+at::Tensor maxpool2x2_nhwc(at::Tensor input, bool emit_pad,
+                           c10::optional<at::Tensor> out_opt) {
     CHECK_GPU(input); CHECK_BF16(input);
     TORCH_CHECK(input.is_contiguous(at::MemoryFormat::ChannelsLast));
     int B = input.size(0), C = input.size(1), H = input.size(2),
         W = input.size(3);
     TORCH_CHECK(C % 8 == 0);
     int Ho = (H + 1) / 2, Wo = (W + 1) / 2;
-    auto out = at::empty({B, C, Ho, Wo},
-                         input.options()
-                             .memory_format(at::MemoryFormat::ChannelsLast));
+    auto out = nhwc_out(input, B, C, Ho, Wo, emit_pad, out_opt);
     int64_t n = (int64_t)B * Ho * Wo * C;
     hipStream_t s = at::cuda::getCurrentCUDAStream();
     hipLaunchKernelGGL(maxpool2x2_nhwc_kernel, dim3(cdiv(n / 8, 256)),
                        dim3(256), 0, s,
                        (const bf16*)input.data_ptr(),
-                       (bf16*)out.data_ptr(), B, H, W, C, Ho, Wo);
+                       (bf16*)out.data_ptr(), B, H, W, C, Ho, Wo,
+                       emit_pad ? 1 : 0);
     HIP_OK(hipGetLastError());
     return out;
 }
@@ -470,7 +450,7 @@
                             const bf16* __restrict__ bias,
                             bf16* __restrict__ out,
                             int M, int Hh, int Ww, int Cin, int Cout,
-                            int relu) {
+                            int relu, int emit_pad) {
     constexpr int BM = 128, BN = 128, BKc = 64;
     __shared__ bf16 lds[2 * BM * BKc];
     bf16* As = lds;
@@ -567,28 +547,47 @@
         __syncthreads();
     }
 
+    const int col0 = bn + wc * 64 + (lane & 15);
+    float bv[4];
 #pragma unroll
     for (int ni = 0; ni < 4; ++ni) {
-        int col = bn + wc * 64 + ni * 16 + (lane & 15);
-        float bv = (bias != nullptr && col < Cout) ? bf2f(bias[col]) : 0.f;
-#pragma unroll
-        for (int mi = 0; mi < 4; ++mi) {
-#pragma unroll
-            for (int r = 0; r < 4; ++r) {
-                int row = bm + wr * 64 + mi * 16 + (lane >> 4) * 4 + r;
+        int col = col0 + ni * 16;
+        bv[ni] = (bias != nullptr && col < Cout) ? bf2f(bias[col]) : 0.f;
+    }
+#pragma unroll
+    for (int mi = 0; mi < 4; ++mi) {
+        const int row0 = bm + wr * 64 + mi * 16 + (lane >> 4) * 4;
+        PadPix pr = {0, 0, 0};
+        if (emit_pad) pr = pad_pix(min(row0, M - 1), Hh, Ww);
+#pragma unroll
+        for (int r = 0; r < 4; ++r) {
+            int row = row0 + r;
+            if (emit_pad && r > 0) pad_pix_next(pr, Hh, Ww);
+            bf16* orow = out + (int64_t)(emit_pad ? pr.pix : row) * Cout;
+#pragma unroll
+            for (int ni = 0; ni < 4; ++ni) {
+                int col = col0 + ni * 16;
                 if (row < M && col < Cout) {
-                    float vv = acc[mi][ni][r] + bv;
+                    float vv = acc[mi][ni][r] + bv[ni];
                     if (relu) vv = fmaxf(vv, 0.f);
-                    out[(int64_t)row * Cout + col] = f2bf(vv);
+                    orow[col] = f2bf(vv);
                 }
             }
         }
     }
+    if (emit_pad) {
+        const int cols[4] = {col0, col0 + 16, col0 + 32, col0 + 48};
+#pragma unroll 1
+        for (int mi = 0; mi < 4; ++mi)
+            pad_border_run(out, bm + wr * 64 + mi * 16 + (lane >> 4) * 4,
+                           M, Hh, Ww, Cout, cols);
+    }
 }
 
 at::Tensor conv_igemm_glds_fwd(at::Tensor padded, at::Tensor w_ohwi,
                                at::Tensor bias, int64_t Hh, int64_t Ww,
-                               bool relu) {
+                               bool relu, bool emit_pad,
+                               c10::optional<at::Tensor> out_opt) {
     CHECK_GPU(padded); CHECK_BF16(padded);
     CHECK_GPU(w_ohwi); CHECK_CONTIG(w_ohwi); CHECK_BF16(w_ohwi);
     TORCH_CHECK(padded.is_contiguous(at::MemoryFormat::ChannelsLast));
@@ -596,9 +595,7 @@
     TORCH_CHECK(padded.size(2) == Hh + 2 && padded.size(3) == Ww + 2);
     int Cout = w_ohwi.size(0);
     TORCH_CHECK(Cin % 64 == 0 && Cout % 8 == 0);
-    auto out = at::empty({B, Cout, Hh, Ww},
-                         padded.options()
-                             .memory_format(at::MemoryFormat::ChannelsLast));
+    auto out = nhwc_out(padded, B, Cout, Hh, Ww, emit_pad, out_opt);
     const bf16* bias_ptr = nullptr;
     if (bias.defined() && bias.numel() > 0)
         bias_ptr = (const bf16*)bias.contiguous().data_ptr();
@@ -609,19 +606,20 @@
                        (const bf16*)padded.data_ptr(),
                        (const bf16*)w_ohwi.data_ptr(), bias_ptr,
                        (bf16*)out.data_ptr(), (int)M, (int)Hh, (int)Ww,
-                       (int)Cin, (int)Cout, relu ? 1 : 0);
+                       (int)Cin, (int)Cout, relu ? 1 : 0,
+                       emit_pad ? 1 : 0);
     HIP_OK(hipGetLastError());
     return out;
 }
 
 
-__global__ __launch_bounds__(256)
+__global__ __launch_bounds__(256, 5)
 void conv_igemm_glds64_kernel(const bf16* __restrict__ inp,
                               const bf16* __restrict__ w,
                               const bf16* __restrict__ bias,
                               bf16* __restrict__ out,
                               int M, int Hh, int Ww, int Cin, int Cout,
-                              int relu) {
+                              int relu, int emit_pad) {
     constexpr int BM = 128, BKc = 64;
     __shared__ bf16 lds[(BM + 64) * BKc];
     bf16* As = lds;
@@ -724,28 +722,47 @@
         __syncthreads();
     }
 
+    const int col0 = bn + (lane & 15);
+    float bv[4];
 #pragma unroll
     for (int ni = 0; ni < 4; ++ni) {
-        int col = bn + ni * 16 + (lane & 15);
-        float bv = (bias != nullptr && col < Cout) ? bf2f(bias[col]) : 0.f;
-#pragma unroll
-        for (int mi = 0; mi < 2; ++mi) {
-#pragma unroll
-            for (int r = 0; r < 4; ++r) {
-                int row = bm + wave * 32 + mi * 16 + (lane >> 4) * 4 + r;
+        int col = col0 + ni * 16;
+        bv[ni] = (bias != nullptr && col < Cout) ? bf2f(bias[col]) : 0.f;
+    }
+#pragma unroll
+    for (int mi = 0; mi < 2; ++mi) {
+        const int row0 = bm + wave * 32 + mi * 16 + (lane >> 4) * 4;
+        PadPix pr = {0, 0, 0};
+        if (emit_pad) pr = pad_pix(min(row0, M - 1), Hh, Ww);
+#pragma unroll
+        for (int r = 0; r < 4; ++r) {
+            int row = row0 + r;
+            if (emit_pad && r > 0) pad_pix_next(pr, Hh, Ww);
+            bf16* orow = out + (int64_t)(emit_pad ? pr.pix : row) * Cout;
+#pragma unroll
+            for (int ni = 0; ni < 4; ++ni) {
+                int col = col0 + ni * 16;
                 if (row < M && col < Cout) {
-                    float vv = acc[mi][ni][r] + bv;
+                    float vv = acc[mi][ni][r] + bv[ni];
                     if (relu) vv = fmaxf(vv, 0.f);
-                    out[(int64_t)row * Cout + col] = f2bf(vv);
+                    orow[col] = f2bf(vv);
                 }
             }
         }
     }
+    if (emit_pad) {
+        const int cols[4] = {col0, col0 + 16, col0 + 32, col0 + 48};
+#pragma unroll 1
+        for (int mi = 0; mi < 2; ++mi)
+            pad_border_run(out, bm + wave * 32 + mi * 16 + (lane >> 4) * 4,
+                           M, Hh, Ww, Cout, cols);
+    }
 }
 
 at::Tensor conv_igemm_glds64_fwd(at::Tensor padded, at::Tensor w_ohwi,
                                  at::Tensor bias, int64_t Hh, int64_t Ww,
-                                 bool relu) {
+                                 bool relu, bool emit_pad,
+                                 c10::optional<at::Tensor> out_opt) {
     CHECK_GPU(padded); CHECK_BF16(padded);
     CHECK_GPU(w_ohwi); CHECK_CONTIG(w_ohwi); CHECK_BF16(w_ohwi);
     TORCH_CHECK(padded.is_contiguous(at::MemoryFormat::ChannelsLast));
@@ -753,9 +770,7 @@
     TORCH_CHECK(padded.size(2) == Hh + 2 && padded.size(3) == Ww + 2);
     int Cout = w_ohwi.size(0);
     TORCH_CHECK(Cin % 64 == 0 && Cout % 8 == 0);
-    auto out = at::empty({B, Cout, Hh, Ww},
-                         padded.options()
-                             .memory_format(at::MemoryFormat::ChannelsLast));
+    auto out = nhwc_out(padded, B, Cout, Hh, Ww, emit_pad, out_opt);
     const bf16* bias_ptr = nullptr;
     if (bias.defined() && bias.numel() > 0)
         bias_ptr = (const bf16*)bias.contiguous().data_ptr();
@@ -766,7 +781,8 @@
                        (const bf16*)padded.data_ptr(),
                        (const bf16*)w_ohwi.data_ptr(), bias_ptr,
                        (bf16*)out.data_ptr(), (int)M, (int)Hh, (int)Ww,
-                       (int)Cin, (int)Cout, relu ? 1 : 0);
+                       (int)Cin, (int)Cout, relu ? 1 : 0,
+                       emit_pad ? 1 : 0);
     HIP_OK(hipGetLastError());
     return out;
 }
diff --git a/sat_amd/ops/csrc/conv8p.hip b/sat_amd/ops/csrc/conv8p.hip
--- a/sat_amd/ops/csrc/conv8p.hip
+++ b/sat_amd/ops/csrc/conv8p.hip
@@ -25,7 +25,7 @@
                           bf16* __restrict__ out,
                           float* __restrict__ outf,
                           int M, int Hh, int Ww, int Cin, int Cout,
-                          int relu, int kt_per) {
+                          int relu, int kt_per, int emit_pad) {
     __shared__ bf16 lds[8 * SLOT];
 
     const int tid = threadIdx.x;
@@ -193,6 +193,23 @@
 #undef A_DELTA
 #undef B_DELTA
 
+    int prow[8][4];
+#pragma unroll
+    for (int i = 0; i < 8; ++i) {
+        const int row0 = bm + (i >> 2) * 128 + wr * 64 + (i & 3) * 16
+            + (lane >> 4) * 4;
+        if (!SPLIT && emit_pad) {
+            PadPix p = pad_pix(min(row0, M - 1), Hh, Ww);
+#pragma unroll
+            for (int r = 0; r < 4; ++r) {
+                if (r) pad_pix_next(p, Hh, Ww);
+                prow[i][r] = p.pix;
+            }
+        } else {
+#pragma unroll
+            for (int r = 0; r < 4; ++r) prow[i][r] = row0 + r;
+        }
+    }
 #pragma unroll
     for (int bH = 0; bH < 2; ++bH) {
 #pragma unroll
@@ -217,8 +234,8 @@
                                 float v = acc[aH * 4 + mi]
                                     [bH * 2 + ni][r] + bv;
                                 if (relu) v = fmaxf(v, 0.f);
-                                out[(int64_t)row * Cout + col]
-                                    = f2bf(v);
+                                out[(int64_t)prow[aH * 4 + mi][r] * Cout
+                                    + col] = f2bf(v);
                             }
                         }
                     }
@@ -226,27 +243,48 @@
             }
         }
     }
+    if (!SPLIT && emit_pad) {
+        const int c0 = bn + wc * 32 + (lane & 15);
+        const int cols[4] = {c0, c0 + 16, c0 + 128, c0 + 144};
+#pragma unroll 1
+        for (int i = 0; i < 8; ++i)
+            pad_border_run(out, bm + (i >> 2) * 128 + wr * 64
+                           + (i & 3) * 16 + (lane >> 4) * 4,
+                           M, Hh, Ww, Cout, cols);
+    }
 }
 
 __global__ void f32_bias_act_nhwc_kernel(const float* __restrict__ yf,
                                          const bf16* __restrict__ bias,
                                          bf16* __restrict__ out,
-                                         int64_t n, int C, int relu) {
+                                         int64_t n, int C, int relu,
+                                         int Hh, int Ww, int emit_pad) {
     int64_t i8 = ((int64_t)blockIdx.x * blockDim.x + threadIdx.x) * 8;
     if (i8 >= n) return;
     int c0 = (int)(i8 % C);
+    bf16x8 o;
 #pragma unroll
     for (int e = 0; e < 8; ++e) {
         float t = yf[i8 + e];
         if (bias != nullptr) t += bf2f(bias[c0 + e]);
         if (relu) t = fmaxf(t, 0.f);
-        out[i8 + e] = f2bf(t);
+        o[e] = f2bf(t);
+    }
+    if (emit_pad) {
+        PadPix pr = pad_pix((int)(i8 / C), Hh, Ww);
+        bf16* op = out + (int64_t)pr.pix * C + c0;
+        *(bf16x8*)op = o;
+        pad_border_zero<bf16x8>(op, pr.y, pr.x, Hh, Ww, C);
+    } else {
+        *(bf16x8*)(out + i8) = o;
     }
 }
 
 at::Tensor conv_igemm_8p_fwd(at::Tensor padded, at::Tensor w_ohwi,
                              at::Tensor bias, int64_t Hh, int64_t Ww,
-                             bool relu) {
+                             bool relu, bool emit_pad,
+                             c10::optional<at::Tensor> out_opt,
+                             int64_t split) {
     CHECK_GPU(padded); CHECK_BF16(padded);
     CHECK_GPU(w_ohwi); CHECK_CONTIG(w_ohwi); CHECK_BF16(w_ohwi);
     TORCH_CHECK(padded.is_contiguous(at::MemoryFormat::ChannelsLast));
@@ -256,9 +294,7 @@
     TORCH_CHECK(Cin % 64 == 0 && Cin >= 64, "conv_igemm_8p: Cin % 64");
     TORCH_CHECK(Cout % 256 == 0, "conv_igemm_8p: Cout % 256");
     TORCH_CHECK(w_ohwi.numel() == (int64_t)Cout * 9 * Cin);
-    auto out = at::empty({B, Cout, Hh, Ww},
-                         padded.options()
-                             .memory_format(at::MemoryFormat::ChannelsLast));
+    auto out = nhwc_out(padded, B, Cout, Hh, Ww, emit_pad, out_opt);
     const bf16* bias_ptr = nullptr;
     if (bias.defined() && bias.numel() > 0)
         bias_ptr = (const bf16*)bias.contiguous().data_ptr();
@@ -268,6 +304,8 @@
     int blocks = cdiv(Cout, 256) * cdiv(M, 256);
     int KT = 9 * (Cin / 64);
     int splitz = std::max(1, std::min({8, 224 / blocks, KT / 2}));
+    if (split >= 0)
+        splitz = std::max(1, std::min((int)split, KT));
     hipStream_t s = at::cuda::getCurrentCUDAStream();
     if (splitz > 1) {
         auto scratch = at::zeros({M, Cout},
@@ -281,13 +319,14 @@
                            (const bf16*)w_ohwi.data_ptr(), bias_ptr,
                            nullptr, (float*)scratch.data_ptr(),
                            M, (int)Hh, (int)Ww,
-                           (int)Cin, (int)Cout, relu ? 1 : 0, kt_per);
+                           (int)Cin, (int)Cout, relu ? 1 : 0, kt_per, 0);
         int64_t n = (int64_t)M * Cout;
         hipLaunchKernelGGL(f32_bias_act_nhwc_kernel,
                            dim3(cdiv(n / 8, 256)), dim3(256), 0, s,
                            (const float*)scratch.data_ptr(), bias_ptr,
                            (bf16*)out.data_ptr(), n, (int)Cout,
-                           relu ? 1 : 0);
+                           relu ? 1 : 0, (int)Hh, (int)Ww,
+                           emit_pad ? 1 : 0);
     } else {
         dim3 grid(cdiv(Cout, 256), cdiv(M, 256));
         hipLaunchKernelGGL((conv_igemm_8p_kernel<0>), grid, dim3(512),
@@ -296,7 +335,8 @@
                            (const bf16*)w_ohwi.data_ptr(), bias_ptr,
                            (bf16*)out.data_ptr(), nullptr,
                            M, (int)Hh, (int)Ww,
-                           (int)Cin, (int)Cout, relu ? 1 : 0, KT);
+                           (int)Cin, (int)Cout, relu ? 1 : 0, KT,
+                           emit_pad ? 1 : 0);
     }
     HIP_OK(hipGetLastError());
     return out;
```

Result: faster. 6003 images/sec, median of 6 (+2.1%).
